# TritonDataCenter/dragnet

Measured on AMD Instinct MI355X. Metric: NDJSON records/sec (whole node), krill filter + 2-field breakdown (req.method,res.statusCode), higher is better.
Workload: dtype uint8; 1 GPU; model=dn scan: filter eq(req.method,GET) + breakdown req.method,res.statusCode, global_batch=4743501, seq_len=226, parallelism=dp1

## Files before the change

dragnet_amd/engine/gpu.py:

```python

import os
import stat
from types import SimpleNamespace

import numpy as np

from . import capacity, decode, xpose
from . import plan as planmod
from .chunks import _pad, choose_chunk_bytes, frame_files
from .decode import (
    C_DS_FAILEDEVAL, C_DS_FILTERED, C_GLOBAL_N, C_INVALID_JSON, C_LINES,
    C_OVERFLOW, C_PARSED, CM_AGG_IN, CM_BADDATE, CM_FAILEDEVAL,
    CM_FILTER_IN, CM_FILTERED, CM_N, CM_NONNUMERIC, CM_TIME_OUT, CM_UNDEF)
from .xpose import _build_xpose_layout


def _env_int(name, default):
    try:
        return int(os.environ.get(name, default))
    except ValueError:
        return default


def first_guess_slots():
    return (_env_int("DRAGNET_AGG_SLOTS", 1 << 20),
            _env_int("DRAGNET_DICT_SLOTS", 1 << 20))


def _is_regular(path):
    try:
        return stat.S_ISREG(os.stat(path).st_mode)
    except OSError:
        return False


class GpuEngine(object):
    name = "gpu"

    def __init__(self, device=None):
        import torch
        self.torch = torch
        if not torch.cuda.is_available():
            raise RuntimeError("no GPU visible (torch.cuda unavailable)")
        from ..ops import load_ops
        self.ops = load_ops(required=True)
        self.device = device if device is not None else \
            torch.device("cuda", torch.cuda.current_device())
        self.chunk_bytes = _env_int("DRAGNET_CHUNK_MB", 256) * 1024 * 1024
        self.coded_stats = {"launches": 0, "retries": 0}
        if self.chunk_bytes > (3 << 30):
            raise ValueError(
                "DRAGNET_CHUNK_MB too large: device chunk addressing "
                "is 32-bit (max 3072 MB per chunk)")


    def scan(self, files, queries, ds_filter=None, time_field=None,
             data_format="json", byte_source=None):
        from ..datasource.file import ScanResult

        cplan = planmod.compile_plan(
            queries, ds_filter=ds_filter, time_field=time_field,
            data_format=data_format)

        agg_slots, dict_slots = first_guess_slots()
        dict_data = _env_int("DRAGNET_DICT_DATA_MB", 256) * 1024 * 1024

        if (byte_source is not None or _env_int("DRAGNET_GROW", 0) == 1
                or not all(_is_regular(p) for p in files)):
            ctx = _ScanContext(self, cplan, agg_slots, dict_slots,
                               dict_data, dense=False, growable=True)
            if byte_source is not None:
                for chunk in byte_source:
                    ctx.feed(chunk)
                ctx.flush()
            else:
                ctx.scan_files(files)
            if ctx.overflowed():
                raise RuntimeError(
                    "table overflow on non-restartable byte source")
            aggs, stages = ctx.finalize(queries)
            return ScanResult(aggs, stages, gpu_stats=dict(
                ctx.planner.grow_counts(), restarts=0))

        dense = None
        nogrow = {"agg": [0] * len(queries), "sdict": 0, "sdata": 0,
                  "ndict": 0}
        for attempt in range(4):
            ctx = _ScanContext(self, cplan, agg_slots, dict_slots,
                               dict_data, dense=dense)
            ctx.scan_files(files)
            if ctx.overflowed():
                from ..log import get_logger
                if ctx.dense:
                    get_logger().child("gpu-engine").warn(
                        "dense directory overflow; restarting on the "
                        "hash path", agg_slots=agg_slots)
                    dense = False
                    continue
                get_logger().child("gpu-engine").warn(
                    "aggregation table overflow; restarting scan",
                    agg_slots=agg_slots * 8, dict_slots=dict_slots * 8)
                dense = False
                agg_slots *= 8
                dict_slots *= 8
                dict_data *= 4
                continue
            aggs, stages = ctx.finalize(queries)
            return ScanResult(aggs, stages,
                              gpu_stats=dict(nogrow, restarts=attempt))
        raise RuntimeError("aggregation tables overflowed after retries")

    def columnar_query(self, query, filt, params, kinds, cols, vals):
        from . import colquery
        return colquery.columnar_query(self, query, filt, params, kinds,
                                       cols, vals)

    def coded_query(self, query, filt, params, kinds, merged,
                    timings=None):
        from . import colquery
        return colquery.coded_query(self, query, filt, params, kinds,
                                    merged, timings)


class _ScanContext(object):
    def __init__(self, eng, cplan, agg_slots, dict_slots, dict_data_cap,
                 dense=None, growable=False):
        torch = eng.torch
        if growable:
            dense = False
        self.eng = eng
        self.t = torch
        self.cplan = cplan
        dev = eng.device
        if dense is None:
            dense = _env_int("DRAGNET_DENSE", 1) == 1
        self.dense = dense
        if dense:
            agg_slots = _env_int("DRAGNET_DENSE_SLOTS", 8192)

        def dev_i32(np_arr):
            return torch.from_numpy(
                np.ascontiguousarray(np_arr.astype(np.int32))).to(dev)

        def dev_f64(np_arr):
            return torch.from_numpy(
                np.ascontiguousarray(np_arr.astype(np.float64))).to(dev)

        progs, bounds = cplan.programs
        metrics, sreq = cplan.metrics
        bds, steps = cplan.breakdown_descs
        plan = dict(
            field_sigs=torch.from_numpy(
                cplan.field_sigs.view(np.int64)).to(dev),
            comp_slot=torch.from_numpy(cplan.comp_slot).to(dev),
            nf_match=cplan.nf_match,
            sig_bloom=cplan.sig_bloom,
            fields_parent_sig=cplan.fields_parent_sig,
            prog_nodes=dev_i32(progs),
            prog_bounds=dev_i32(bounds),
            const_meta=dev_i32(cplan.const_meta),
            const_dvals=dev_f64(cplan.const_dvals),
            const_bytes=torch.from_numpy(
                np.ascontiguousarray(cplan.const_bytes)).to(dev),
            synth_slots=dev_i32(cplan.synthetic),
            n_synth=cplan.n_synth,
            metric_rows=dev_i32(metrics),
            synth_req=dev_i32(sreq),
            bd_rows=dev_i32(bds),
            bd_steps=dev_f64(steps),
            value_slot=cplan.value_slot,
            fields_slot=cplan.fields_slot,
            skinner=cplan.data_format == "json-skinner",
        )

        self.state = eng.ops.ScanState(
            plan=plan, agg_slots=agg_slots, dict_slots=dict_slots,
            dict_data_bytes=dict_data_cap, dense=dense)

        self.planner = None
        if growable:
            nm, s_cols, n_cols = capacity.plan_shape(metrics, bds)
            sizes = self.state.sizes()
            self.planner = capacity.CapacityPlanner(
                nm, s_cols, n_cols,
                dict(sizes, agg=[sizes["agg%d" % m] for m in range(nm)]))

        self._pinned = self._dev_data = None
        self._pos = self._nlines = self._segs = None
        self._partial = b""
        self._copy_ev = None
        self._fin_stream = None
        self._files = None
        self._pool = None
        self._x = None

    @property
    def counters(self):
        return self.state.counters

    @property
    def agg_slots(self):
        return max(v for k, v in self.state.sizes().items()
                   if k.startswith("agg"))

    @property
    def dict_slots(self):
        sizes = self.state.sizes()
        return max(sizes["sdict"], sizes["ndict"])


    def feed(self, chunk):
        data = self._partial + chunk
        cut = data.rfind(b"\n")
        if cut < 0:
            self._partial = data
            return
        self._partial = data[cut + 1:]
        self._run(data[:cut + 1])

    def flush(self):
        if self._partial:
            self._run(self._partial + b"\n")
            self._partial = b""

    def _ensure_buffers(self, padded):
        torch = self.t
        dev = self.eng.device
        if self._pinned is not None and self._pinned.numel() >= padded:
            return
        cap = max(padded, self.eng.chunk_bytes + (1 << 20))
        cap = (cap + 15) & ~15
        self._pinned = torch.empty(cap, dtype=torch.uint8, pin_memory=True)
        self._dev_data = torch.empty(cap, dtype=torch.uint8, device=dev)
        self._pos = torch.empty(cap + 2, dtype=torch.int32, device=dev)
        self._nlines = torch.zeros(1, dtype=torch.int32, device=dev)
        self._segs = torch.empty(cap // 2048 + 2, dtype=torch.int32,
                                 device=dev)

    @staticmethod
    def _pad_pinned(pin, n):
        padded = _pad(n)
        pin[n:padded] = 10
        return padded

    def _index(self, dev_data, start, end):
        self.eng.ops.newline_index(dev_data, start, end, self._segs,
                                   self._pos, self._nlines)
        return self._pos, self._nlines

    def _submit(self, dev_data, start, end, index=None):
        pos, nlines = index or self._index(dev_data, start, end)
        if self.planner is None:
            self.state.scan(dev_data, pos, nlines, start)
        else:
            self._scan_planned(dev_data, pos, nlines, start, end)


    def _scan_planned(self, dev_data, pos, nlines, start, end):
        torch = self.t
        pl = self.planner
        g = pl.floor
        host = torch.cat(
            [nlines, pos[g - 1:end - start:g]]).cpu().numpy()
        nrec = min(int(host[0]), pos.numel())
        marks = host[1:].view(np.uint32)

        def start_of(i):
            if i == 0:
                return start
            if i == nrec:
                return end
            return int(marks[i // g - 1]) + 1

        a = 0
        while a < nrec:
            b = pl.next_range(a, nrec, start_of, self._measure, self.grow)
            self.state.scan(dev_data, pos[a:b], nlines, start_of(a))
            a = b

    def _measure(self, names):
        occ = self.state.occupancy().cpu().tolist()
        true = dict(zip(self.planner.names, occ))
        return {n: true[n] for n in names}

    def grow(self, name, new_size):
        old = self.planner.size[name]
        if name.startswith("agg"):
            self.state.grow_agg(int(name[3:]), new_size)
        else:
            getattr(self.state, "grow_" + name)(new_size)
        self.planner.size[name] = new_size
        from ..log import get_logger
        get_logger().child("gpu-engine").warn(
            "table grown in place", structure=name, size=old,
            new_size=new_size)

    def _run(self, buf):
        torch = self.t
        n = len(buf)
        self._ensure_buffers(_pad(n))
        pin = self._pinned
        if self._copy_ev is None:
            self._copy_ev = torch.cuda.Event()
        else:
            self._copy_ev.synchronize()
        pin[:n] = torch.frombuffer(bytearray(buf), dtype=torch.uint8)
        padded = self._pad_pinned(pin, n)
        self._dev_data[:padded].copy_(pin[:padded], non_blocking=True)
        self._copy_ev.record()
        self._submit(self._dev_data, 0, n)

    def overflowed(self):
        return int(self.counters[C_OVERFLOW].item()) > 0


    def scan_files(self, files):
        cap = self.eng.chunk_bytes
        if self._pinned is None:
            try:
                total = sum(os.stat(p).st_size for p in files)
            except OSError:
                total = 0
            cap = choose_chunk_bytes(total, cap,
                                     "DRAGNET_CHUNK_MB" in os.environ)
        pins = self._ensure_file_staging(cap)
        evs = [None, None]

        def wait(i):
            if evs[i] is not None:
                evs[i].synchronize()
                evs[i] = None

        frames = frame_files(files, [memoryview(p.numpy()) for p in pins],
                             cap, wait, _env_int("DRAGNET_READERS", 24))
        try:
            for i, n in frames:
                evs[i] = self._run_pinned(pins[i], n)
        finally:
            frames.close()

    def _ensure_file_staging(self, cap):
        torch = self.t
        if self._files is None:
            if self._pinned is None:
                self._ensure_buffers(_pad(cap))
            self._files = SimpleNamespace(
                pins=[self._pinned, torch.empty(
                    self._pinned.numel(), dtype=torch.uint8,
                    pin_memory=True)],
                copy_stream=torch.cuda.Stream(device=self.eng.device),
                dev=[self._dev_data, torch.empty_like(self._dev_data)],
                done=[torch.cuda.Event(), torch.cuda.Event()],
                idx=0)
        return self._files.pins

    def _run_pinned(self, pin, n):
        torch = self.t
        f = self._files
        padded = self._pad_pinned(pin, n)
        idx = f.idx
        f.idx ^= 1
        dev_data = f.dev[idx]
        main = torch.cuda.current_stream(self.eng.device)
        cs = f.copy_stream
        cs.wait_event(f.done[idx])
        ev = torch.cuda.Event()
        with torch.cuda.stream(cs):
            dev_data[:padded].copy_(pin[:padded], non_blocking=True)
            ev.record(cs)
        main.wait_event(ev)
        self._submit(dev_data, 0, n)
        f.done[idx].record(main)
        return ev


    def stage_resident(self, buf, n_slices=None):
        torch = self.t
        if n_slices is None:
            n_slices = _env_int("DRAGNET_SLICES", 6)
        n = len(buf)
        self._ensure_buffers(_pad(n))
        pin = self._pinned
        pin[:n] = torch.frombuffer(bytearray(buf), dtype=torch.uint8)
        padded = self._pad_pinned(pin, n)

        bounds = sorted({0, n} | {buf.rfind(b"\n", 0, n * k // n_slices) + 1
                                  for k in range(1, n_slices)})
        slices = list(zip(bounds, bounds[1:]))
        self._pool = p = SimpleNamespace(
            n=n, padded=padded, slices=slices,
            copy_stream=torch.cuda.Stream(device=self.eng.device),
            evs=[torch.cuda.Event() for _ in slices],
            dev_pp=torch.empty_like(self._dev_data),
            pass_done=[torch.cuda.Event(), torch.cuda.Event()],
            idx=0, pos=[])

        self._dev_data[:padded].copy_(pin[:padded])
        for (s, e) in slices:
            pos, nlines = self._index(self._dev_data, s, e)
            p.pos.append(
                (pos[:int(nlines.item())].clone(), nlines.clone()))

    def scan_resident(self, h2d=True):
        torch = self.t
        p = self._pool
        padded = p.padded
        dev_data = self._dev_data
        pin = self._pinned
        main = torch.cuda.current_stream(self.eng.device)
        if h2d:
            idx = p.idx
            p.idx ^= 1
            dev_data = self._dev_data if idx == 0 else p.dev_pp
            ev_done = p.pass_done[idx]
            p.copy_stream.wait_event(ev_done)
            with torch.cuda.stream(p.copy_stream):
                for k, (s, e) in enumerate(p.slices):
                    s16 = s & ~15
                    e16 = min((e + 15) & ~15, padded)
                    dev_data[s16:e16].copy_(pin[s16:e16],
                                            non_blocking=True)
                    p.evs[k].record(p.copy_stream)
        for k, (s, e) in enumerate(p.slices):
            if h2d:
                main.wait_event(p.evs[k])
                self._submit(dev_data, s, e)
            else:
                self._submit(dev_data, s, e, p.pos[k])
        if h2d:
            ev_done.record(main)


    def stage_xpose(self, buf=None):
        gran = _env_int("DRAGNET_XGRAN", 64)
        if gran not in (32, 64, 128):
            raise ValueError("DRAGNET_XGRAN must be 32, 64 or 128")
        if os.environ.get("DRAGNET_XPOSE_HOST") == "1":
            self._x = xpose.build_on_host(self.t, buf, gran,
                                          self.eng.device)
            return
        if self._pool is None:
            if buf is None:
                raise ValueError("no resident pool to transpose")
            self.stage_resident(buf)
        pos, nlines = self._index(self._dev_data, 0, self._pool.n)
        self._x = xpose.build_on_device(self.t, self.eng.ops,
                                        self._dev_data, pos, nlines, gran)

    def scan_xpose(self):
        self.state.scan_xpose(*self._x)

    def make_graph(self, h2d=True, xpose=False):
        torch = self.t

        def pass_():
            self.reset()
            if xpose:
                self.scan_xpose()
            else:
                self.scan_resident(h2d=h2d)

        try:
            pass_()
            torch.cuda.synchronize(self.eng.device)
            g = torch.cuda.CUDAGraph()
            with torch.cuda.graph(g):
                pass_()
            torch.cuda.synchronize(self.eng.device)
            return g
        except Exception:
            return None

    def reset(self):
        self.state.reset()
        if self.planner is not None:
            self.planner.occ = dict.fromkeys(self.planner.names, 0)


    def finalize(self, queries):
        return self.decode_extracted(self.extract_async(queries),
                                     queries)

    def extract_async(self, queries):
        h = self.state.extract_all()
        h["ev"] = self.t.cuda.Event()
        h["ev"].record()
        return h

    def decode_extracted(self, h, queries):
        torch = self.t
        if self._fin_stream is None:
            self._fin_stream = torch.cuda.Stream(device=self.eng.device)
        with torch.cuda.stream(self._fin_stream):
            self._fin_stream.wait_event(h["ev"])
            host = {"cnt": h["cnt"].cpu().numpy()}
            host.update(self._fetch_dicts(h))
            host["aggs"] = []
            for k_full, c_full, out_n in h["aggs"][:len(queries)]:
                n_out = min(int(out_n.item()), k_full.shape[0])
                host["aggs"].append((k_full[:n_out].cpu().numpy(),
                                     c_full[:n_out].cpu().numpy()))
        return decode.decode_snapshot(host, queries, self.cplan)

    @staticmethod
    def _fetch_dicts(h):
        n_str = int(h["n_str"].item())
        n_num = int(h["n_num"].item())
        host = {"n_str": n_str, "n_num": n_num}
        if n_str:
            host["str_off"] = h["str_off"][:n_str].cpu().numpy()
            host["str_len"] = h["str_len"][:n_str].cpu().numpy()
            used = int(h["used"].item())
            host["blob"] = h["blob"][:used].cpu().numpy()
        if n_num:
            host["numbers"] = h["numbers"][:n_num].cpu().numpy()
        return host

    @classmethod
    def _decode_dicts(cls, h):
        return decode.decode_dicts(cls._fetch_dicts(h))
```

dragnet_amd/engine/plan.py:

```python


import os

import numpy as np

from .. import krill

FNV_OFFSET = 0xCBF29CE484222325
FNV_PRIME = 0x100000001B3
MASK64 = (1 << 64) - 1

OP_AND = 0
OP_OR = 1
OP_EQ = 2
OP_NE = 3
OP_LT = 4
OP_LE = 5
OP_GT = 6
OP_GE = 7
OP_TRUE = 8

CONST_NUM = 0
CONST_STR = 1
CONST_NULL = 2

BUCKET_NONE = 0
BUCKET_P2 = 1
BUCKET_LIN = 2

MAX_FIELDS = 24
MAX_DEPTH = 12
MAX_KEY = 8

(M_PROG, M_NBD, M_BD_OFF, M_NSYNTH, M_SYNTH_OFF, M_HAS_TF, M_T_GE,
 M_T_LT) = range(8)
M_N = 8


def fnv1a(data, h=FNV_OFFSET):
    for b in data:
        h = ((h ^ b) * FNV_PRIME) & MASK64
    return h


def _mix64(x):
    x &= MASK64
    x ^= x >> 33
    x = (x * 0xFF51AFD7ED558CCD) & MASK64
    x ^= x >> 33
    x = (x * 0xC4CEB9FE1A85EC53) & MASK64
    x ^= x >> 33
    return x


SIG_LENK = 0xFF51AFD7ED558CCD
SIG_LIT_MARK = 0xC2B2AE3D27D4EB4F


def _sig_mix(x):
    x &= MASK64
    x ^= x >> 32
    x = (x * 0xD6E8FEB86659FD93) & MASK64
    return x ^ (x >> 32)


def comp_into(sig, b):
    for k in range(0, len(b), 8):
        w = int.from_bytes(b[k:k + 8].ljust(8, b"\0"), "little")
        sig = _sig_mix(sig ^ w)
    return _sig_mix(sig ^ ((len(b) * SIG_LENK) & MASK64))


def lit_sig(name):
    return comp_into(FNV_OFFSET, name.encode("utf-8"))


def path_sig(path):
    sig = FNV_OFFSET
    for comp in path.split("."):
        sig = comp_into(sig, comp.encode("utf-8"))
    return sig


class PlanError(Exception):
    pass


class FieldTable(object):
    def __init__(self, prefix=""):
        self.prefix = prefix
        self.paths = []
        self.by_path = {}

    def slot(self, path, raw=False):
        key = (path, raw)
        if key in self.by_path:
            return self.by_path[key]
        i = len(self.paths)
        if i >= MAX_FIELDS:
            raise PlanError(
                "query references more than %d fields" % MAX_FIELDS)
        self.paths.append(key)
        self.by_path[key] = i
        return i

    def sigs(self):
        return np.array(
            [path_sig(p if raw else self.prefix + p)
             for p, raw in self.paths],
            dtype=np.uint64)


class ConstPool(object):
    def __init__(self):
        self.metas = []
        self.dvals = []
        self.bytes = bytearray()

    def add(self, v):
        if v is None:
            self.metas.append((CONST_NULL, 0, 0, 0))
            self.dvals.append(0.0)
        elif isinstance(v, bool):
            self.metas.append((CONST_NUM, 0, 0, 1))
            self.dvals.append(1.0 if v else 0.0)
        elif isinstance(v, (int, float)):
            self.metas.append((CONST_NUM, 0, 0, 1))
            self.dvals.append(float(v))
        else:
            import json as _json
            b = v.encode("utf-8")
            off = len(self.bytes)
            self.bytes.extend(b)
            num = krill.to_number(v)
            valid = 0 if num != num else 1
            esc = _json.dumps(v, ensure_ascii=False)[1:-1].encode("utf-8")
            if esc != b:
                off2 = len(self.bytes)
                self.bytes.extend(esc)
                alt = (off2, len(esc))
            else:
                alt = (0, 0)
            self.metas.append((CONST_STR, off, len(b), valid) + alt)
            self.dvals.append(num if valid else 0.0)
            return len(self.metas) - 1
        self.metas.append(self.metas.pop() + (0, 0))
        return len(self.metas) - 1


def compile_predicate(pred, fields, consts):
    nodes = []

    def emit(p):
        idx = len(nodes)
        if len(p) == 0:
            nodes.append([OP_TRUE, 0, 0, idx + 1])
            return
        (key, val), = p.items()
        if key == "and" or key == "or":
            nodes.append([OP_AND if key == "and" else OP_OR,
                          len(val), 0, 0])
            for sub in val:
                emit(sub)
            nodes[idx][3] = len(nodes)
            return
        op = {"eq": OP_EQ, "ne": OP_NE, "lt": OP_LT,
              "le": OP_LE, "gt": OP_GT, "ge": OP_GE}[key]
        slot = fields.slot(val[0])
        cidx = consts.add(val[1])
        nodes.append([op, slot, cidx, idx + 1])

    emit(pred if pred is not None else {})
    return nodes


class CompiledPlan(object):

    def __init__(self, fields, programs, const_meta, const_dvals,
                 const_bytes, synthetic, metrics, breakdown_descs,
                 queries):
        self.fields = fields
        self.field_sigs = fields.sigs()
        self.programs = programs
        self.const_meta = const_meta
        self.const_dvals = const_dvals
        self.const_bytes = const_bytes
        self.synthetic = synthetic
        self.metrics = metrics
        self.breakdown_descs = breakdown_descs
        self.queries = queries

    def describe(self):
        return {
            "fields": list(self.fields.paths),
            "n_metrics": int(self.metrics[0].shape[0]),
        }


def compile_plan(queries, ds_filter=None, time_field=None,
                 data_format="json"):
    prefix = "fields." if data_format == "json-skinner" else ""
    fields = FieldTable(prefix)
    consts = ConstPool()
    prog_nodes = []
    prog_bounds = []

    def add_program(pred):
        start = len(prog_nodes)
        nodes = compile_predicate(pred, fields, consts)
        for n in nodes:
            n[3] += start
        prog_nodes.extend(nodes)
        prog_bounds.append((start, len(prog_nodes)))
        return len(prog_bounds) - 1

    ds_prog = add_program(ds_filter)

    synth_slots = []
    synth_by_slot = {}

    def synth_index(src_path):
        slot = fields.slot(src_path)
        if slot in synth_by_slot:
            return synth_by_slot[slot]
        synth_by_slot[slot] = len(synth_slots)
        synth_slots.append(slot)
        return synth_by_slot[slot]

    metric_rows = []
    bd_rows = []
    bd_steps = []
    synth_req = []

    for q in queries:
        if len(q.breakdowns) > MAX_KEY:
            raise PlanError(
                "query has more than %d breakdowns (GPU key width); "
                "use the CPU engine" % MAX_KEY)
        prog_id = add_program(q.filter)

        my_synth = []
        for b in q.breakdowns:
            if "date" in b:
                my_synth.append(synth_index(b["field"]))
        has_tf = 0
        t_ge = t_lt = 0
        dn_ts_idx = -1
        if q.before_ms is not None:
            if not time_field:
                raise PlanError(
                    'datasource is missing "timefield" for "before" '
                    'and "after" constraints')
            dn_ts_idx = synth_index(time_field)
            my_synth.append(dn_ts_idx)
            has_tf = 1
            t_ge = -(-q.after_ms // 1000)
            t_lt = -(-q.before_ms // 1000)

        sreq_off = len(synth_req)
        seen = set()
        my_synth_u = [s for s in my_synth
                      if not (s in seen or seen.add(s))]
        synth_req.extend(my_synth_u)

        synth_names = {b["name"]: b["field"]
                       for b in q.breakdowns if "date" in b}
        if q.time_field:
            synth_names.setdefault(q.time_field, q.time_field)

        bd_off = len(bd_rows)
        for b in q.breakdowns:
            if "date" in b:
                kind = 1
                ref = synth_index(b["field"])
            elif b["name"] in synth_names:
                kind = 1
                ref = synth_index(synth_names[b["name"]])
            else:
                kind = 0
                ref = fields.slot(b["name"])
            bk = q.bucketizers.get(b["name"])
            if bk is None:
                bkind, step = BUCKET_NONE, 0.0
            elif bk.aggr == "quantize":
                bkind, step = BUCKET_P2, 0.0
            else:
                bkind, step = BUCKET_LIN, float(bk.step)
            bd_rows.append([kind, ref, bkind, 0])
            bd_steps.append(step)

        row = {M_PROG: prog_id, M_NBD: len(q.breakdowns),
               M_BD_OFF: bd_off, M_NSYNTH: len(my_synth_u),
               M_SYNTH_OFF: sreq_off, M_HAS_TF: has_tf,
               M_T_GE: int(t_ge), M_T_LT: int(t_lt)}
        metric_rows.append([row[c] for c in range(M_N)])

    value_slot = -1
    fields_slot = -1
    if data_format == "json-skinner":
        value_slot = fields.slot("value", raw=True)
        fields_slot = fields.slot("fields", raw=True)

    nf_match = len(fields.paths)
    comp_slot = np.full(max(nf_match, 1), -1, dtype=np.int32)
    comp_sigs = []
    no_companions = os.environ.get("DRAGNET_NO_COMPANIONS") == "1"
    if data_format != "json-skinner" and not no_companions:
        for i, (pth, raw) in enumerate(fields.paths):
            if not raw and "." in pth:
                phys = nf_match + len(comp_sigs)
                if phys >= MAX_FIELDS:
                    raise PlanError(
                        "query references more than %d fields "
                        "(incl. dotted-key companions)" % MAX_FIELDS)
                comp_slot[i] = phys
                comp_sigs.append(lit_sig(pth))
    elif data_format == "json-skinner" and not no_companions:
        for i, (pth, raw) in enumerate(fields.paths):
            if not raw and "." in pth:
                phys = nf_match + len(comp_sigs)
                if phys >= MAX_FIELDS:
                    raise PlanError(
                        "query references more than %d fields "
                        "(incl. dotted-key companions)" % MAX_FIELDS)
                comp_slot[i] = phys
                comp_sigs.append(_sig_mix(
                    path_sig(prefix + pth) ^ SIG_LIT_MARK))

    programs = np.array(prog_nodes, dtype=np.int32).reshape(-1, 4)
    bounds = np.array(prog_bounds, dtype=np.int32).reshape(-1, 2)
    const_meta = np.array(consts.metas, dtype=np.int32).reshape(-1, 6)
    const_dvals = np.array(consts.dvals, dtype=np.float64)
    const_bytes = np.frombuffer(
        bytes(consts.bytes) or b"\0", dtype=np.uint8).copy()
    synthetic = np.array(synth_slots or [0], dtype=np.int32)
    metrics = np.array(metric_rows, dtype=np.int32).reshape(-1, M_N)
    bds = np.array(bd_rows or [[0, 0, 0, 0]],
                   dtype=np.int32).reshape(-1, 4)
    steps = np.array(bd_steps or [0.0], dtype=np.float64)
    sreq = np.array(synth_req or [0], dtype=np.int32)

    plan = CompiledPlan(
        fields, (programs, bounds), const_meta, const_dvals,
        const_bytes, synthetic, (metrics, sreq), (bds, steps), queries)
    plan.n_synth = len(synth_slots)
    plan.comp_slot = comp_slot
    plan.nf_match = nf_match
    bloom = 0
    for sg in ([int(x) for x in fields.sigs()] + comp_sigs):
        bloom |= 1 << (sg & 63)
    plan.sig_bloom = bloom - (1 << 64) if bloom >= (1 << 63) else bloom
    if comp_sigs:
        plan.field_sigs = np.concatenate(
            [plan.field_sigs,
             np.array(comp_sigs, dtype=np.uint64)])
    plan.value_slot = value_slot
    plan.fields_slot = fields_slot
    fps = path_sig("fields") if data_format == "json-skinner" else 0
    plan.fields_parent_sig = fps - (1 << 64) if fps >= (1 << 63) else fps
    plan.ds_prog = ds_prog
    plan.data_format = data_format
    return plan



TAG_ORD = 0
TAG_STR = 1
TAG_NUM = 2
TAG_SPECIAL = 3
ORD_BIAS = 1 << 29
SPECIAL_NULL = 0
SPECIAL_UNDEF = 1
SPECIAL_TRUE = 2
SPECIAL_FALSE = 3
SPECIAL_OBJECT = 4
SPECIAL_ARRAY = 5
SPECIAL_ARRJSON = 6
EMPTY_CODE = 0xFFFFFFFF


def decode_key(codes, query, strings, numbers):
    from ..points import js_num_str
    out = []
    for b, code in zip(query.breakdowns, codes):
        tag = code >> 30
        val = code & 0x3FFFFFFF
        bk = query.bucketizers.get(b["name"])
        if bk is not None:
            if tag == TAG_ORD:
                out.append(int(val) - ORD_BIAS)
            else:
                assert tag == TAG_NUM
                out.append(int(numbers[val]))
        elif tag == TAG_STR:
            out.append(strings[val])
        elif tag == TAG_NUM:
            num = numbers[val]
            if "date" in b:
                out.append(int(num))
            else:
                out.append(js_num_str(
                    int(num) if float(num).is_integer()
                    and abs(num) < 2**53 else float(num)))
        elif tag == TAG_SPECIAL:
            if (val & 7) == SPECIAL_ARRJSON:
                import json as _json
                from ..points import js_array_str
                raw = strings[val >> 3]
                try:
                    out.append(js_array_str(_json.loads(raw)))
                except ValueError:
                    out.append(raw)
            else:
                out.append({
                    SPECIAL_NULL: "null", SPECIAL_UNDEF: "undefined",
                    SPECIAL_TRUE: "true", SPECIAL_FALSE: "false",
                    SPECIAL_OBJECT: "[object Object]",
                    SPECIAL_ARRAY: "<array>"}[val])
        else:
            raise PlanError("bad code tag %d" % tag)
    return tuple(out)
```

dragnet_amd/ops/hip/common.h:

```cpp
#pragma once
#if defined(__HIPCC__)
#include <hip/hip_runtime.h>
#endif
#include <cstddef>
#include <cstdint>
#include "hd.h"

namespace dn {

constexpr int MAX_FIELDS = 24;
constexpr int MAX_DEPTH  = 64;
constexpr int SLOT_DEPTH = 12;
constexpr int MAX_KEY    = 8;
constexpr int MAX_SYNTH  = 8;
constexpr int PRED_STACK = 8;

enum PredOp : int32_t {
  OP_AND = 0, OP_OR = 1,
  OP_EQ = 2, OP_NE = 3, OP_LT = 4, OP_LE = 5, OP_GT = 6, OP_GE = 7,
  OP_TRUE = 8,
};

enum ConstKind : int32_t { CONST_NUM = 0, CONST_STR = 1, CONST_NULL = 2 };

enum BucketKind : int32_t { BUCKET_NONE = 0, BUCKET_P2 = 1, BUCKET_LIN = 2 };

enum FieldType : uint8_t {
  T_MISSING = 0, T_NULL = 1, T_FALSE = 2, T_TRUE = 3,
  T_NUM = 4, T_STR = 5, T_OBJ = 6, T_ARR = 7,
};

constexpr uint32_t TAG_ORD     = 0u;
constexpr uint32_t TAG_STR     = 1u;
constexpr uint32_t TAG_NUM     = 2u;
constexpr uint32_t TAG_SPECIAL = 3u;
constexpr uint32_t ORD_BIAS    = 1u << 29;
constexpr uint32_t SPECIAL_NULL = 0, SPECIAL_UNDEF = 1,
                   SPECIAL_TRUE = 2, SPECIAL_FALSE = 3,
                   SPECIAL_OBJECT = 4, SPECIAL_ARRAY = 5,
                   SPECIAL_ARRJSON = 6;
constexpr uint32_t EMPTY_CODE = 0xFFFFFFFFu;

inline DN_HD uint32_t make_code(uint32_t tag, uint32_t val) {
  return (tag << 30) | (val & 0x3FFFFFFFu);
}

enum CounterSlot : int {
  C_LINES = 0,
  C_INVALID_JSON = 1,
  C_PARSED = 2,
  C_DS_FILTERED = 3,
  C_DS_FAILEDEVAL = 4,
  C_OVERFLOW = 5,
  C_GLOBAL_N = 8,
  CM_FILTER_IN = 0, CM_FILTERED = 1, CM_FAILEDEVAL = 2,
  CM_UNDEF = 3, CM_BADDATE = 4, CM_TIME_OUT = 5,
  CM_AGG_IN = 6, CM_NONNUMERIC = 7,
  CM_N = 8,
};

constexpr uint32_t SLOT_EMPTY = 0, SLOT_CLAIMED = 1, SLOT_READY = 2;

struct AggTable {
  uint32_t* state;
  uint32_t* keys;
  double*   count;
  uint32_t  nslots;
  double*   partial;
  uint32_t  prows;
  uint32_t  pad_;
};

struct StrDict {
  uint32_t* state;
  uint64_t* hash;
  uint32_t* id;
  uint32_t* off;
  uint32_t* len;
  uint32_t  nslots;
  uint8_t*  data;
  uint32_t  data_cap;
  uint32_t* data_used;
  uint32_t* next_id;
};

struct NumDict {
  uint32_t* state;
  uint64_t* bits;
  uint32_t* id;
  uint32_t  nslots;
  uint32_t* next_id;
};


struct PlanView {
  const uint64_t* field_sigs;
  int nf;
  const int32_t* comp_slot;
  int nf_match;
  uint64_t sig_bloom;
  const int32_t* prog_nodes;
  const int32_t* prog_bounds;
  const int32_t* const_meta;
  const double*  const_dvals;
  const uint8_t* const_bytes;
  const int32_t* synth_slots;
  int ns;
  const int32_t* metric_rows;
  const int32_t* synth_req;
  const int32_t* bd_rows;
  const double*  bd_steps;
  int nm;
  int value_slot;
  int fields_slot;
  uint64_t fields_parent_sig;
};

struct ScanArgs {
  const uint8_t* data;
  const uint32_t* nl_pos;
  const uint32_t* nlines_ptr;
  uint32_t pos_cap;
  uint32_t first_start;
  uint32_t tile_cap;
  PlanView P;
  AggTable* tables;
  StrDict sdict;
  NumDict ndict;
  unsigned long long* counters;
  int data_format_skinner;
  const uint8_t* xdata;
  const unsigned long long* xwave_base;
  const uint32_t* xrec_len;
  uint32_t xn_slots;
};

}
```

dragnet_amd/ops/hip/ext.hip:

```cpp

#include <torch/extension.h>
#include <cstdlib>
#include <cstring>
#include <c10/hip/HIPStream.h>

#include "scan_kernels.hip"

namespace dn {

namespace {

#define CHECK_GPU(t) TORCH_CHECK((t).is_cuda(), #t " must be on GPU")

constexpr size_t LDS_MAX = 160 * 1024;

hipStream_t current_stream() {
  return c10::hip::getCurrentHIPStream().stream();
}

template <class... KArgs, class... Args>
void launch(const char* what, void (*kernel)(KArgs...), dim3 grid,
            dim3 block, size_t lds, Args&&... args) {
  hipLaunchKernelGGL(kernel, grid, block, lds, current_stream(),
                     std::forward<Args>(args)...);
  hipError_t err = hipGetLastError();
  TORCH_CHECK(err == hipSuccess, what, " launch failed: ",
              hipGetErrorString(err));
}

constexpr uint32_t GRID_CAP = 2048;

uint32_t grid_for(uint64_t n) {
  return (uint32_t)std::min<uint64_t>((n + BLOCK - 1) / BLOCK, GRID_CAP);
}

int env_int(const char* name, int dflt) {
  const char* v = getenv(name);
  return v ? atoi(v) : dflt;
}

size_t lds_bytes(int64_t nf, int64_t nm, int64_t ns, bool columnar) {
  return LdsLayout((int)nf, (int)nm, columnar ? 0 : (int)ns, !columnar)
      .total;
}

using ScanKernel = void (*)(ScanArgs);

ScanKernel linear_kernel(int mw) {
  switch (mw) {
    case 2: return scan_kernel_mw<2>;
    case 3: return scan_kernel_mw<3>;
    case 4: return scan_kernel_mw<4>;
    case 5: return scan_kernel_mw<5>;
    case 6: return scan_kernel_mw<6>;
    default: return scan_kernel;
  }
}

ScanKernel xpose_kernel(int mw, int xg) {
  if (xg == 32) return scan_kernel_x<4, 5>;
  if (xg == 128) return scan_kernel_x<4, 7>;
  switch (mw) {
    case 2: return scan_kernel_x<2, 6>;
    case 3: return scan_kernel_x<3, 6>;
    case 5: return scan_kernel_x<5, 6>;
    default: return scan_kernel_x<4, 6>;
  }
}

}

void newline_index(torch::Tensor data, int64_t start, int64_t n,
                   torch::Tensor seg_scratch,
                   torch::Tensor pos_out, torch::Tensor total_out) {
  CHECK_GPU(data);
  int64_t span = n - (start & ~(int64_t)15);
  uint32_t nseg = (uint32_t)((span + NL_SEG - 1) / NL_SEG);
  TORCH_CHECK((int64_t)nseg <= seg_scratch.numel(),
              "seg_scratch too small");
  if (span <= 0) {
    total_out.zero_();
    return;
  }
  const uint8_t* d = (const uint8_t*)data.data_ptr();
  uint32_t* segs = (uint32_t*)seg_scratch.data_ptr();
  uint32_t blocks = (nseg + 3) / 4;
  launch("newline_count", newline_count_kernel, dim3(blocks), dim3(256), 0,
         d, (uint32_t)start, (uint32_t)n, segs, nseg);
  launch("newline_scan", newline_scan_kernel, dim3(1), dim3(1024), 0,
         segs, nseg, (uint32_t*)total_out.data_ptr());
  launch("newline_write", newline_write_kernel, dim3(blocks), dim3(256), 0,
         d, (uint32_t)start, (uint32_t)n, segs, nseg,
         (uint32_t*)pos_out.data_ptr(), (uint32_t)pos_out.numel());
}

torch::Tensor col_descs_host(std::vector<int64_t> kinds,
                             std::vector<torch::Tensor> nums,
                             std::vector<torch::Tensor> soffs,
                             std::vector<torch::Tensor> slens) {
  int nf = (int)kinds.size();
  auto out = torch::zeros({(long)(nf * sizeof(ColDesc))},
                          torch::dtype(torch::kUInt8));
  ColDesc* d = (ColDesc*)out.data_ptr();
  for (int f = 0; f < nf; f++) {
    d[f].kind = (int32_t)kinds[f];
    d[f].num = kinds[f] == COL_NUM ? (const double*)nums[f].data_ptr()
                                   : nullptr;
    d[f].soff = (kinds[f] == COL_STR || kinds[f] == COL_CODED)
                    ? (const uint32_t*)soffs[f].data_ptr()
                    : nullptr;
    d[f].slen = kinds[f] == COL_STR ? (const uint32_t*)slens[f].data_ptr()
                                    : nullptr;
  }
  return out;
}

void xpose_build(torch::Tensor data, torch::Tensor sstart,
                 torch::Tensor slen, torch::Tensor wbase,
                 int64_t n_slots, int64_t gran_log, torch::Tensor xb) {
  CHECK_GPU(data);
  CHECK_GPU(xb);
  uint32_t nw = (uint32_t)(n_slots >> 6);
  TORCH_CHECK(wbase.numel() >= (long)nw + 1, "wbase needs nw+1 rows");
  uint32_t blocks = (nw + 3) / 4;
  launch("xpose_build", xpose_build_kernel, dim3(blocks), dim3(256), 0,
         (const uint8_t*)data.data_ptr(),
         (const uint32_t*)sstart.data_ptr(),
         (const uint32_t*)slen.data_ptr(),
         (const unsigned long long*)wbase.data_ptr(),
         (uint32_t)n_slots, (int)gran_log, (uint8_t*)xb.data_ptr());
}

class ScanState {
 public:
  ScanState(py::dict plan, int64_t agg_slots, int64_t dict_slots,
            int64_t dict_data_bytes, bool dense)
      : dense_(dense) {
    auto ptr = [&](py::dict& d, const char* key) {
      owned_.push_back(py::cast<torch::Tensor>(d[key]));
      return owned_.back().data_ptr();
    };
    PlanView& P = args_.P;
    P.field_sigs = (const uint64_t*)ptr(plan, "field_sigs");
    P.nf = (int)owned_.back().numel();
    P.comp_slot = (const int32_t*)ptr(plan, "comp_slot");
    P.nf_match = py::cast<int>(plan["nf_match"]);
    P.sig_bloom = (uint64_t)py::cast<int64_t>(plan["sig_bloom"]);
    P.prog_nodes = (const int32_t*)ptr(plan, "prog_nodes");
    P.prog_bounds = (const int32_t*)ptr(plan, "prog_bounds");
    P.const_meta = (const int32_t*)ptr(plan, "const_meta");
    P.const_dvals = (const double*)ptr(plan, "const_dvals");
    P.const_bytes = (const uint8_t*)ptr(plan, "const_bytes");
    P.synth_slots = (const int32_t*)ptr(plan, "synth_slots");
    P.ns = py::cast<int>(plan["n_synth"]);
    P.metric_rows = (const int32_t*)ptr(plan, "metric_rows");
    P.nm = (int)(owned_.back().numel() / 8);
    P.synth_req = (const int32_t*)ptr(plan, "synth_req");
    P.bd_rows = (const int32_t*)ptr(plan, "bd_rows");
    P.bd_steps = (const double*)ptr(plan, "bd_steps");
    P.value_slot = py::cast<int>(plan["value_slot"]);
    P.fields_slot = py::cast<int>(plan["fields_slot"]);
    P.fields_parent_sig =
        (uint64_t)py::cast<int64_t>(plan["fields_parent_sig"]);
    args_.data_format_skinner = py::cast<bool>(plan["skinner"]) ? 1 : 0;

    for (auto& t : owned_) CHECK_GPU(t);
    device_ = owned_.front().device();

    check_slots(agg_slots, "agg table", AGG_LOG2);
    check_slots(dict_slots, "sdict", DICT_LOG2);
    check_bytes(dict_data_bytes);
    states_.resize(P.nm);
    keys_.resize(P.nm);
    counts_.resize(P.nm);
    if (dense_) partials_.resize(P.nm);
    for (int m = 0; m < P.nm; m++) alloc_agg(m, agg_slots);
    alloc_sdict(dict_slots);
    alloc_ndict(dict_slots);
    sd_data_ = zeros({dict_data_bytes}, U8);
    sd_used_ = zeros({1}, I32);
    sd_next_ = zeros({1}, I32);
    nd_next_ = zeros({1}, I32);
    counters_ = zeros({C_GLOBAL_N + P.nm * CM_N}, I64);
    bind_tables();
    bind_dicts();
    args_.counters = (unsigned long long*)counters_.data_ptr();

    int mw = env_int("DRAGNET_MIN_WAVES", 4);
    linear_ = linear_kernel(mw);
    xpose_ = xpose_kernel(mw, env_int("DRAGNET_XGRAN", 64));

    lds_ = lds_bytes(P.nf, P.nm, P.ns, false);
    TORCH_CHECK(lds_ <= LDS_MAX, "plan needs too much LDS: ", lds_);
    int tile_req = env_int("DRAGNET_LDS_STAGE", 0);
    if (tile_req != 0) {
      size_t avail = (LDS_MAX - lds_ - 256) & ~(size_t)15;
      tile_cap_ = (tile_req < 0) ? avail
                                 : std::min((size_t)tile_req, avail);
      if (tile_cap_ > 100 * 1024) tile_cap_ = 100 * 1024;
      if (tile_cap_ < 24 * 1024) tile_cap_ = 0;
    }
    args_.tile_cap = (uint32_t)tile_cap_;
  }

  void scan(torch::Tensor data, torch::Tensor nl_pos,
            torch::Tensor nlines, int64_t first_start) {
    CHECK_GPU(data);
    CHECK_GPU(nl_pos);
    ScanArgs A = args_;
    A.data = (const uint8_t*)data.data_ptr();
    A.nl_pos = (const uint32_t*)nl_pos.data_ptr();
    A.nlines_ptr = (const uint32_t*)nlines.data_ptr();
    A.pos_cap = (uint32_t)nl_pos.numel();
    A.first_start = (uint32_t)first_start;
    launch("scan_kernel", linear_, dim3(grid_for(A.pos_cap)), dim3(BLOCK),
           lds_ + tile_cap_, A);
  }

  void scan_xpose(torch::Tensor xdata, torch::Tensor wave_base,
                  torch::Tensor rec_len, int64_t n_slots) {
    CHECK_GPU(xdata);
    TORCH_CHECK(n_slots > 0, "empty transposed staging");
    ScanArgs A = args_;
    A.xdata = (const uint8_t*)xdata.data_ptr();
    A.xwave_base = (const unsigned long long*)wave_base.data_ptr();
    A.xrec_len = (const uint32_t*)rec_len.data_ptr();
    A.xn_slots = (uint32_t)n_slots;
    launch("scan_kernel_x", xpose_, dim3(grid_for(A.xn_slots)),
           dim3(BLOCK), lds_ + tile_cap_, A);
  }

  void columnar_query(torch::Tensor col_descs, torch::Tensor blob,
                      torch::Tensor values, int64_t nrows,
                      std::vector<torch::Tensor> columns) {
    ColumnLaunch L = bind_columns("columnar", col_descs, blob, values,
                                  nrows, std::move(columns));
    if (L.blocks == 0) return;
    launch("columnar_query", columnar_query_kernel, dim3(L.blocks),
           dim3(BLOCK), L.lds, L.A);
  }

  void coded_query(torch::Tensor col_descs, torch::Tensor dict_blob,
                   torch::Tensor doff, torch::Tensor dlen,
                   torch::Tensor seg_start, torch::Tensor values,
                   int64_t nrows, std::vector<torch::Tensor> columns) {
    for (auto* t : {&doff, &dlen, &seg_start}) CHECK_GPU(*t);
    TORCH_CHECK(doff.numel() == dlen.numel(), "doff / dlen differ");
    TORCH_CHECK(doff.numel() < (int64_t)0xFFFFFFFFll, "dictionary too big");
    TORCH_CHECK(seg_start.numel() >= 2 &&
                    seg_start.numel() - 1 < (int64_t)ORD_BIAS,
                "seg_start needs nfiles + 1 entries");
    ColumnLaunch L = bind_columns("coded", col_descs, dict_blob, values,
                                  nrows, std::move(columns));
    auto code2id = zeros({std::max<int64_t>(doff.numel(), 1)}, I32);
    col_inputs_.insert(col_inputs_.end(),
                       {doff, dlen, seg_start, code2id});
    CodedArgs X;
    X.ndict = (uint32_t)doff.numel();
    X.nfiles = (uint32_t)(seg_start.numel() - 1);
    X.doff = (const uint32_t*)doff.data_ptr();
    X.dlen = (const uint32_t*)dlen.data_ptr();
    X.code2id = (const uint32_t*)code2id.data_ptr();
    X.seg_start = (const uint32_t*)seg_start.data_ptr();
    if (X.ndict > 0)
      launch("dict_intern", dict_intern_kernel,
             dim3((X.ndict + 255) / 256), dim3(256), 0, L.A.sdict, L.A.blob,
             X.doff, X.dlen, X.ndict, (uint32_t*)code2id.data_ptr(),
             overflow_ptr());
    if (L.blocks == 0) return;
    launch("coded_query", coded_query_kernel, dim3(L.blocks), dim3(BLOCK),
           L.lds, L.A, X);
  }

  void reset() {
    hipStream_t st = current_stream();
    auto z = [&](torch::Tensor& t) {
      hipError_t e = hipMemsetAsync(t.data_ptr(), 0,
                                    (size_t)t.numel() * t.element_size(),
                                    st);
      TORCH_CHECK(e == hipSuccess, "reset memset failed: ",
                  hipGetErrorString(e));
    };
    for (auto& t : states_) z(t);
    for (auto& t : counts_) z(t);
    for (auto& t : partials_) z(t);
    z(sd_state_); z(sd_used_); z(sd_next_);
    z(nd_state_); z(nd_next_); z(counters_);
  }

  py::dict extract_all() {
    for (const AggTable& T : tables_) dense_reduce(T);
    const StrDict& sd = args_.sdict;
    const NumDict& nd = args_.ndict;
    py::dict out;
    out["cnt"] = counters_.clone();
    out["n_str"] = sd_next_.clone();
    out["n_num"] = nd_next_.clone();
    out["used"] = sd_used_.clone();
    out["blob"] = sd_data_.clone();

    long n_sids = std::max<long>(sd.nslots, 1);
    auto str_off = zeros({n_sids}, I32);
    auto str_len = zeros({n_sids}, I32);
    if (sd.nslots > 0)
      launch("extract_strdict", extract_strdict_kernel,
             dim3((sd.nslots + 255) / 256), dim3(256), 0, sd,
             (uint32_t*)str_off.data_ptr(), (uint32_t*)str_len.data_ptr(),
             sd.nslots);
    out["str_off"] = str_off;
    out["str_len"] = str_len;

    auto numbers = zeros({std::max<long>(nd.nslots, 1)}, F64);
    if (nd.nslots > 0)
      launch("extract_numdict", extract_numdict_kernel,
             dim3((nd.nslots + 255) / 256), dim3(256), 0, nd,
             (double*)numbers.data_ptr(), nd.nslots);
    out["numbers"] = numbers;

    py::list aggs;
    for (const AggTable& T : tables_) {
      long max_out = T.nslots;
      auto out_keys = zeros({max_out, (long)MAX_KEY}, I32);
      auto out_counts = zeros({max_out}, F64);
      auto out_n = zeros({1}, I32);
      launch("extract_agg", extract_agg_kernel,
             dim3((T.nslots + 255) / 256), dim3(256), 0, T,
             (uint32_t*)out_keys.data_ptr(),
             (double*)out_counts.data_ptr(), (uint32_t*)out_n.data_ptr(),
             (uint32_t)max_out);
      aggs.append(py::make_tuple(out_keys, out_counts, out_n));
    }
    out["aggs"] = aggs;
    return out;
  }

  py::dict sizes() const {
    py::dict out;
    for (size_t m = 0; m < tables_.size(); m++)
      out[py::str("agg" + std::to_string(m))] = tables_[m].nslots;
    out["sdict"] = args_.sdict.nslots;
    out["sdata"] = args_.sdict.data_cap;
    out["ndict"] = args_.ndict.nslots;
    return out;
  }

  torch::Tensor counters() const { return counters_; }


  torch::Tensor occupancy() {
    std::vector<torch::Tensor> parts;
    for (auto& st : states_)
      parts.push_back(st.eq((int64_t)SLOT_READY).sum().reshape({1}));
    for (auto* t : {&sd_next_, &sd_used_, &nd_next_})
      parts.push_back(t->to(torch::kInt64));
    return torch::cat(parts);
  }

  void grow_agg(int64_t m, int64_t new_slots) {
    TORCH_CHECK(!dense_, "dense tables do not grow");
    TORCH_CHECK(m >= 0 && (size_t)m < tables_.size(), "no such metric");
    AggTable old = tables_[m];
    check_slots(new_slots, "agg table", AGG_LOG2, old.nslots);
    std::vector<torch::Tensor> keep = {states_[m], keys_[m], counts_[m]};
    growing("agg" + std::to_string(m), old.nslots, new_slots,
            [&] { alloc_agg(m, new_slots); });
    bind_tables();
    launch("rehash_agg", rehash_agg_kernel, dim3((old.nslots + 255) / 256),
           dim3(256), 0, old, tables_[m], overflow_ptr());
  }

  void grow_sdict(int64_t new_slots) {
    StrDict old = args_.sdict;
    check_slots(new_slots, "sdict", DICT_LOG2, old.nslots);
    std::vector<torch::Tensor> keep = {sd_state_, sd_hash_, sd_id_,
                                       sd_off_, sd_len_};
    growing("sdict", old.nslots, new_slots, [&] { alloc_sdict(new_slots); });
    bind_dicts();
    launch("rehash_strdict", rehash_strdict_kernel,
           dim3((old.nslots + 255) / 256), dim3(256), 0, old, args_.sdict,
           overflow_ptr());
  }

  void grow_sdata(int64_t new_bytes) {
    torch::Tensor old = sd_data_;
    check_bytes(new_bytes, old.numel());
    growing("sdata", old.numel(), new_bytes,
            [&] { sd_data_ = zeros({new_bytes}, U8); });
    bind_dicts();
    hipError_t e = hipMemcpyAsync(
        sd_data_.data_ptr(), old.data_ptr(), (size_t)old.numel(),
        hipMemcpyDeviceToDevice, current_stream());
    TORCH_CHECK(e == hipSuccess, "payload copy failed: ",
                hipGetErrorString(e));
  }

  void grow_ndict(int64_t new_slots) {
    NumDict old = args_.ndict;
    check_slots(new_slots, "ndict", DICT_LOG2, old.nslots);
    std::vector<torch::Tensor> keep = {nd_state_, nd_bits_, nd_id_};
    growing("ndict", old.nslots, new_slots, [&] { alloc_ndict(new_slots); });
    bind_dicts();
    launch("rehash_numdict", rehash_numdict_kernel,
           dim3((old.nslots + 255) / 256), dim3(256), 0, old, args_.ndict,
           overflow_ptr());
  }

 private:
  static constexpr auto I32 = torch::kInt32, I64 = torch::kInt64,
                        F64 = torch::kFloat64, U8 = torch::kUInt8;

  torch::Tensor zeros(at::IntArrayRef shape, torch::ScalarType dtype) const {
    return torch::zeros(shape, torch::dtype(dtype).device(device_));
  }

  static constexpr int DICT_LOG2 = 31, AGG_LOG2 = 29;
  static void check_slots(int64_t n, const char* what, int max_log2,
                          int64_t old = 0) {
    TORCH_CHECK(n > 0 && (n & (n - 1)) == 0 && (n >> max_log2) <= 1, what,
                ": slot count must be a power of two <= 2^", max_log2);
    TORCH_CHECK(n > old, "a table may only grow (", old, " -> ", n,
                " slots)");
  }

  static void check_bytes(int64_t n, int64_t old = -1) {
    TORCH_CHECK(n <= (int64_t)0xFFFFFFFFll,
                "string payload buffer exceeds 32-bit offsets");
    TORCH_CHECK(n > old, "string payload buffer may only grow");
  }

  template <class Alloc>
  static void growing(const std::string& name, int64_t old_size,
                      int64_t new_size, Alloc&& alloc) {
    try {
      alloc();
    } catch (const c10::OutOfMemoryError& e) {
      std::string why = e.what_without_backtrace();
      TORCH_CHECK(false, "cannot grow ", name, " from ", old_size, " to ",
                  new_size, ": device allocation failed (",
                  why.substr(0, why.find('\n')), ")");
    }
  }

  struct ColumnLaunch {
    ColArgs A;
    size_t lds;
    uint32_t blocks;
  };

  ColumnLaunch bind_columns(const char* what, torch::Tensor col_descs,
                            torch::Tensor blob, torch::Tensor values,
                            int64_t nrows,
                            std::vector<torch::Tensor> columns) {
    for (auto* t : {&col_descs, &blob, &values}) CHECK_GPU(*t);
    for (auto& t : columns) {
      CHECK_GPU(t);
      TORCH_CHECK(t.numel() >= nrows, "column shorter than nrows");
    }
    TORCH_CHECK(nrows >= 0 && nrows < (int64_t)0xFFFFFFFFll, what,
                " query: row count exceeds 32 bits");
    TORCH_CHECK(values.numel() >= nrows, "values shorter than nrows");
    ColumnLaunch L;
    ColArgs& A = L.A;
    A.P = column_plan();
    TORCH_CHECK(col_descs.numel() == (int64_t)(A.P.nf * sizeof(ColDesc)),
                "col_descs does not match the plan's field count");
    L.lds = lds_bytes(A.P.nf, A.P.nm, 0, true);
    TORCH_CHECK(L.lds <= LDS_MAX, what, " plan needs too much LDS");
    A.nrows = (uint32_t)nrows;
    A.values = (const double*)values.data_ptr();
    A.blob = (const uint8_t*)blob.data_ptr();
    A.cols = (const ColDesc*)col_descs.data_ptr();
    A.tables = args_.tables;
    A.sdict = args_.sdict;
    A.ndict = args_.ndict;
    A.counters = args_.counters;
    col_inputs_ = std::move(columns);
    col_inputs_.insert(col_inputs_.end(), {col_descs, blob, values});
    L.blocks = grid_for((uint64_t)nrows);
    return L;
  }

  PlanView column_plan() const {
    PlanView P = args_.P;
    P.sig_bloom = 0;
    P.fields_parent_sig = 0;
    P.ns = 0;
    P.value_slot = -1;
    P.fields_slot = -1;
    return P;
  }

  unsigned long long* overflow_ptr() {
    return (unsigned long long*)counters_.data_ptr() + C_OVERFLOW;
  }

  void alloc_agg(size_t m, int64_t n) {
    std::tie(states_[m], keys_[m], counts_[m]) = std::make_tuple(
        zeros({n}, I32), zeros({n * MAX_KEY}, I32), zeros({n}, F64));
    if (dense_) partials_[m] = zeros({GRID_CAP, n}, F64);
  }

  void alloc_sdict(int64_t n) {
    std::tie(sd_state_, sd_hash_, sd_id_, sd_off_, sd_len_) =
        std::make_tuple(zeros({n}, I32), zeros({n}, I64), zeros({n}, I32),
                        zeros({n}, I32), zeros({n}, I32));
  }

  void alloc_ndict(int64_t n) {
    std::tie(nd_state_, nd_bits_, nd_id_) =
        std::make_tuple(zeros({n}, I32), zeros({n}, I64), zeros({n}, I32));
  }

  void bind_dicts() {
    StrDict& sd = args_.sdict;
    sd.state = (uint32_t*)sd_state_.data_ptr();
    sd.hash = (uint64_t*)sd_hash_.data_ptr();
    sd.id = (uint32_t*)sd_id_.data_ptr();
    sd.off = (uint32_t*)sd_off_.data_ptr();
    sd.len = (uint32_t*)sd_len_.data_ptr();
    sd.nslots = (uint32_t)sd_state_.numel();
    sd.data = (uint8_t*)sd_data_.data_ptr();
    sd.data_cap = (uint32_t)sd_data_.numel();
    sd.data_used = (uint32_t*)sd_used_.data_ptr();
    sd.next_id = (uint32_t*)sd_next_.data_ptr();
    NumDict& nd = args_.ndict;
    nd.state = (uint32_t*)nd_state_.data_ptr();
    nd.bits = (uint64_t*)nd_bits_.data_ptr();
    nd.id = (uint32_t*)nd_id_.data_ptr();
    nd.nslots = (uint32_t)nd_state_.numel();
    nd.next_id = (uint32_t*)nd_next_.data_ptr();
  }

  void bind_tables() {
    size_t nm = states_.size();
    tables_.resize(nm);
    for (size_t m = 0; m < nm; m++) {
      AggTable& t = tables_[m];
      t.state = (uint32_t*)states_[m].data_ptr();
      t.keys = (uint32_t*)keys_[m].data_ptr();
      t.count = (double*)counts_[m].data_ptr();
      t.nslots = (uint32_t)states_[m].numel();
      t.partial = dense_ ? (double*)partials_[m].data_ptr() : nullptr;
      t.prows = dense_ ? GRID_CAP : 0;
      t.pad_ = 0;
    }
    auto host = torch::empty({(long)(nm * sizeof(AggTable))},
                             torch::dtype(torch::kUInt8));
    memcpy(host.data_ptr(), tables_.data(), nm * sizeof(AggTable));
    table_descs_ = host.to(device_);
    args_.tables = (AggTable*)table_descs_.data_ptr();
  }

  static void dense_reduce(const AggTable& T) {
    if (T.partial == nullptr || T.prows == 0) return;
    uint32_t tiles = (T.nslots + 15) / 16;
    uint32_t splits = 32;
    while (splits > 1 && T.prows / splits < 16) splits /= 2;
    uint32_t rows_per_blk = (T.prows + splits - 1) / splits;
    rows_per_blk = (rows_per_blk + 3) & ~3u;
    launch("mfma_reduce", mfma_reduce_kernel, dim3(tiles, splits),
           dim3(64), 0, T, rows_per_blk);
  }

  std::vector<torch::Tensor> states_, keys_, counts_, partials_, owned_;
  std::vector<torch::Tensor> col_inputs_;
  torch::Tensor sd_state_, sd_hash_, sd_id_, sd_off_, sd_len_;
  torch::Tensor sd_data_, sd_used_, sd_next_;
  torch::Tensor nd_state_, nd_bits_, nd_id_, nd_next_;
  torch::Tensor counters_, table_descs_;
  c10::Device device_ = c10::kCPU;
  const bool dense_;
  ScanArgs args_ = {};
  std::vector<AggTable> tables_;
  ScanKernel linear_ = nullptr, xpose_ = nullptr;
  size_t lds_ = 0, tile_cap_ = 0;
};

}

PYBIND11_MODULE(TORCH_EXTENSION_NAME, m) {
  m.doc() = "dragnet_amd MI355X scan engine (gfx950 HIP kernels)";
  m.def("newline_index", &dn::newline_index, "device-side newline index");
  m.def("xpose_build", &dn::xpose_build, "device-side wave transpose");
  m.def("col_descs_host", &dn::col_descs_host);
  m.def("lds_bytes", &dn::lds_bytes, py::arg("nf"), py::arg("nm"),
        py::arg("ns") = 0, py::arg("columnar") = false,
        "dynamic LDS bytes of a scan / columnar launch (host only)");
  py::class_<dn::ScanState>(m, "ScanState")
      .def(py::init<py::dict, int64_t, int64_t, int64_t, bool>(),
           py::kw_only(), py::arg("plan"), py::arg("agg_slots"),
           py::arg("dict_slots"), py::arg("dict_data_bytes"),
           py::arg("dense"))
      .def("scan", &dn::ScanState::scan, py::arg("data"),
           py::arg("nl_pos"), py::arg("nlines"), py::arg("first_start"),
           "fused NDJSON scan over one chunk")
      .def("scan_xpose", &dn::ScanState::scan_xpose, py::arg("xdata"),
           py::arg("wave_base"), py::arg("rec_len"), py::arg("n_slots"))
      .def("columnar_query", &dn::ScanState::columnar_query,
           py::arg("col_descs"), py::arg("blob"), py::arg("values"),
           py::arg("nrows"), py::arg("columns"),
           "K7: query over uploaded index columns")
      .def("coded_query", &dn::ScanState::coded_query,
           py::arg("col_descs"), py::arg("dict_blob"), py::arg("doff"),
           py::arg("dlen"), py::arg("seg_start"), py::arg("values"),
           py::arg("nrows"), py::arg("keep"),
           "query over merged dictionary-coded sidecar columns")
      .def("reset", &dn::ScanState::reset)
      .def("extract_all", &dn::ScanState::extract_all)
      .def("occupancy", &dn::ScanState::occupancy,
           "device int64 [ready slots per metric..., string ids, "
           "payload bytes, number ids]")
      .def("sizes", &dn::ScanState::sizes)
      .def_property_readonly("counters", &dn::ScanState::counters)
      .def("grow_agg", &dn::ScanState::grow_agg, py::arg("metric"),
           py::arg("new_slots"),
           "rehash one metric's table into a larger zeroed one")
      .def("grow_sdict", &dn::ScanState::grow_sdict, py::arg("new_slots"))
      .def("grow_sdata", &dn::ScanState::grow_sdata, py::arg("new_bytes"))
      .def("grow_ndict", &dn::ScanState::grow_ndict, py::arg("new_slots"));
  m.attr("MAX_KEY") = (int)dn::MAX_KEY;
  m.attr("MAX_FIELDS") = (int)dn::MAX_FIELDS;
}
```

dragnet_amd/ops/hip/hd.h:

```cpp
#pragma once

#if defined(__HIPCC__)
#define DN_HD __host__ __device__
#define DN_HD_INLINE __host__ __device__ __forceinline__
#define DN_HD_NOINLINE __host__ __device__ __attribute__((noinline))
#else
#define DN_HD
#define DN_HD_INLINE inline
#define DN_HD_NOINLINE __attribute__((noinline))
#endif

#if defined(__HIP_DEVICE_COMPILE__)
#define DN_FFSLL(x) __ffsll(x)
#define DN_DOUBLE_AS_LL(x) __double_as_longlong(x)
#define DN_LL_AS_DOUBLE(x) __longlong_as_double(x)
#define DN_TID() ((uint32_t)threadIdx.x)
#define DN_CONST_TABLE __device__ __constant__
#else
#define DN_FFSLL(x) __builtin_ffsll((long long)(x))
#define DN_DOUBLE_AS_LL(x) __builtin_bit_cast(long long, (double)(x))
#define DN_LL_AS_DOUBLE(x) __builtin_bit_cast(double, (long long)(x))
#define DN_TID() 0u
#define DN_CONST_TABLE static const
#endif
```

dragnet_amd/ops/hip/scan_kernels.hip:

```cpp

#include "common.h"
#include <hip/hip_runtime.h>

extern "C++" {
#include "scan_text.h"
#include "scan_record.h"
#include "scan_tables.h"

namespace dn {

typedef double dn_d4 __attribute__((ext_vector_type(4)));

__global__ void mfma_reduce_kernel(AggTable T, uint32_t rows_per_blk) {
  uint32_t slot0 = blockIdx.x * 16;
  uint32_t r0 = blockIdx.y * rows_per_blk;
  uint32_t r1 = r0 + rows_per_blk;
  if (r1 > T.prows) r1 = T.prows;
  int l = threadIdx.x;
  uint32_t n = slot0 + (l & 15);
  dn_d4 acc = {0.0, 0.0, 0.0, 0.0};
  const double* P = T.partial;
  size_t stride = T.nslots;
  for (uint32_t rt = r0; rt < r1; rt += 4) {
    uint32_t rr = rt + (uint32_t)(l >> 4);
    double b = (rr < r1 && n < T.nslots)
                   ? P[(size_t)rr * stride + n] : 0.0;
    acc = __builtin_amdgcn_mfma_f64_16x16x4f64(1.0, b, acc, 0, 0, 0);
  }
  if (l < 16 && n < T.nslots) {
    double v = acc[0];
    if (v != 0.0) atomicAdd(&T.count[n], v);
  }
}


constexpr uint32_t NL_SEG = 2048;

DEV uint32_t nl_mask32(uint32_t w) {
  uint32_t x = w ^ 0x0A0A0A0Au;
  uint32_t y = (x & 0x7F7F7F7Fu) + 0x7F7F7F7Fu;
  return ~(y | x | 0x7F7F7F7Fu);
}

DEV uint32_t range_mask32(uint32_t wpos, uint32_t start, uint32_t n) {
  uint32_t m = 0x80808080u;
  if (wpos >= start && wpos + 4 <= n) return m;
  uint32_t out = 0;
#pragma unroll
  for (int b = 0; b < 4; b++) {
    uint32_t pos = wpos + b;
    if (pos >= start && pos < n) out |= 0x80u << (b * 8);
  }
  return out;
}

__global__ void newline_count_kernel(const uint8_t* data,
                                     uint32_t start, uint32_t n,
                                     uint32_t* seg_counts,
                                     uint32_t nseg) {
  uint32_t seg = blockIdx.x * (blockDim.x >> 6) + (threadIdx.x >> 6);
  if (seg >= nseg) return;
  uint32_t lane = threadIdx.x & 63u;
  const uint4* p16 = reinterpret_cast<const uint4*>(data);
  uint32_t base0 = (start & ~15u) + seg * NL_SEG;
  uint32_t cnt = 0;
#pragma unroll
  for (int half = 0; half < 2; half++) {
    uint32_t base = base0 + half * 1024u + lane * 16u;
    if (base < n) {
      uint4 v = p16[base >> 4];
      uint32_t w[4] = {v.x, v.y, v.z, v.w};
#pragma unroll
      for (int wi = 0; wi < 4; wi++)
        cnt += __popc(nl_mask32(w[wi]) &
                      range_mask32(base + wi * 4, start, n));
    }
  }
  for (int off = 32; off; off >>= 1) cnt += __shfl_down(cnt, off, 64);
  if (lane == 0) seg_counts[seg] = cnt;
}

__global__ void newline_scan_kernel(uint32_t* seg_counts, uint32_t nseg,
                                    uint32_t* total_out) {
  __shared__ uint32_t tile[1024];
  __shared__ uint32_t carry;
  if (threadIdx.x == 0) carry = 0;
  __syncthreads();
  for (uint32_t base = 0; base < nseg; base += 1024) {
    uint32_t i = base + threadIdx.x;
    uint32_t v = (i < nseg) ? seg_counts[i] : 0;
    tile[threadIdx.x] = v;
    __syncthreads();
    for (uint32_t d = 1; d < 1024; d <<= 1) {
      uint32_t t = (threadIdx.x >= d) ? tile[threadIdx.x - d] : 0;
      __syncthreads();
      tile[threadIdx.x] += t;
      __syncthreads();
    }
    uint32_t incl = tile[threadIdx.x];
    if (i < nseg) seg_counts[i] = carry + incl - v;
    __syncthreads();
    if (threadIdx.x == 1023) carry += tile[1023];
    __syncthreads();
  }
  if (threadIdx.x == 0) *total_out = carry;
}

__global__ void newline_write_kernel(const uint8_t* data,
                                     uint32_t start, uint32_t n,
                                     const uint32_t* seg_offsets,
                                     uint32_t nseg, uint32_t* out_pos,
                                     uint32_t cap) {
  uint32_t seg = blockIdx.x * (blockDim.x >> 6) + (threadIdx.x >> 6);
  if (seg >= nseg) return;
  uint32_t lane = threadIdx.x & 63u;
  const uint4* p16 = reinterpret_cast<const uint4*>(data);
  uint32_t base0 = (start & ~15u) + seg * NL_SEG;
  uint32_t w_at = seg_offsets[seg];
#pragma unroll
  for (int half = 0; half < 2; half++) {
    uint32_t base = base0 + half * 1024u + lane * 16u;
    uint32_t m[4] = {0, 0, 0, 0};
    uint32_t cnt = 0;
    if (base < n) {
      uint4 v = p16[base >> 4];
      uint32_t w[4] = {v.x, v.y, v.z, v.w};
#pragma unroll
      for (int wi = 0; wi < 4; wi++) {
        m[wi] = nl_mask32(w[wi]) &
                range_mask32(base + wi * 4, start, n);
        cnt += __popc(m[wi]);
      }
    }
    uint32_t incl = cnt;
    for (int off = 1; off < 64; off <<= 1) {
      uint32_t t = __shfl_up(incl, off, 64);
      if ((int)lane >= off) incl += t;
    }
    uint32_t at = w_at + incl - cnt;
#pragma unroll
    for (int wi = 0; wi < 4; wi++) {
      uint32_t mm = m[wi];
      while (mm) {
        uint32_t b = ((uint32_t)__ffs(mm) - 1) >> 3;
        if (at < cap) out_pos[at] = base + wi * 4 + b;
        at++;
        mm &= mm - 1;
      }
    }
    w_at += __shfl(incl, 63, 64);
  }
}

__global__ void xpose_build_kernel(const uint8_t* __restrict__ data,
                                   const uint32_t* __restrict__ sstart,
                                   const uint32_t* __restrict__ slen,
                                   const unsigned long long* __restrict__ wbase,
                                   uint32_t n_slots, int gran_log,
                                   uint8_t* __restrict__ xb) {
  uint32_t w = blockIdx.x * (blockDim.x >> 6) + (threadIdx.x >> 6);
  uint32_t nw = n_slots >> 6;
  if (w >= nw) return;
  uint32_t lane = threadIdx.x & 63u;
  uint32_t r = (w << 6) + lane;
  uint32_t gran = 1u << gran_log;
  unsigned long long base = wbase[w];
  uint32_t gw = (uint32_t)((wbase[w + 1] - base) >> (6 + gran_log));
  uint32_t len = slen[r];
  if (len == 0xFFFFFFFFu) len = 0;
  uint32_t start = sstart[r];
  uint8_t* dst0 = xb + base + ((size_t)lane << gran_log);
  for (uint32_t g = 0; g < gw; g++) {
    uint8_t* dst = dst0 + ((size_t)g << (6 + gran_log));
    uint32_t off = g << gran_log;
    for (uint32_t k = 0; k < gran; k += 16) {
      uint8_t tmp[16];
#pragma unroll
      for (int t = 0; t < 16; t++) {
        uint32_t o = off + k + t;
        tmp[t] = (o < len) ? data[start + o] : (uint8_t)'\n';
      }
      uint4 vv;
      __builtin_memcpy(&vv, tmp, 16);
      *reinterpret_cast<uint4*>(dst + k) = vv;
    }
  }
}

template <int XP>
DEV void scan_kernel_body(char* smem, ScanArgs A);

__launch_bounds__(BLOCK)
__global__ void scan_kernel(ScanArgs A) {
  extern __shared__ __attribute__((aligned(16))) char smem0[];
  scan_kernel_body<0>(smem0, A);
}

template <int MW>
__launch_bounds__(BLOCK, MW)
__global__ void scan_kernel_mw(ScanArgs A) {
  extern __shared__ __attribute__((aligned(16))) char smem1[];
  scan_kernel_body<0>(smem1, A);
}
template __global__ void scan_kernel_mw<2>(ScanArgs);
template __global__ void scan_kernel_mw<3>(ScanArgs);
template __global__ void scan_kernel_mw<4>(ScanArgs);
template __global__ void scan_kernel_mw<5>(ScanArgs);
template __global__ void scan_kernel_mw<6>(ScanArgs);

template <int MW, int XLG>
__launch_bounds__(BLOCK, MW)
__global__ void scan_kernel_x(ScanArgs A) {
  extern __shared__ __attribute__((aligned(16))) char smem2[];
  scan_kernel_body<XLG>(smem2, A);
}
template __global__ void scan_kernel_x<2, 6>(ScanArgs);
template __global__ void scan_kernel_x<3, 6>(ScanArgs);
template __global__ void scan_kernel_x<4, 6>(ScanArgs);
template __global__ void scan_kernel_x<5, 6>(ScanArgs);
template __global__ void scan_kernel_x<4, 5>(ScanArgs);
template __global__ void scan_kernel_x<4, 7>(ScanArgs);

#define synth_val_at(si) synth_lds[(si) * BLOCK + threadIdx.x]

template <class BS>
DEV void process_record(BS BV, uint32_t start, uint32_t end,
                        const ScanArgs& A, const PlanView& P, FV& fv,
                        unsigned long long* lcnt, LdsCacheEntry* cache,
                        uint64_t* sig_lds, double* synth_lds) {
  const int nf = P.nf;
  uint32_t synth_ok = 0;
  atomicAdd(&lcnt[C_LINES], 1ull);
  for (int f = 0; f < nf; f++)
    fv.type[f * BLOCK + fv.tid] = T_MISSING;

  uint8_t top_type;
  bool ok = (end > start) &&
            parse_record(BV, start, end, P, fv, top_type, sig_lds,
                         A.data_format_skinner);
  double weight = 1.0;
  if (ok && A.data_format_skinner) {
    bool has_fields = P.fields_slot >= 0 &&
                      fv.get_type(P.fields_slot) != T_MISSING;
    bool val_num = P.value_slot >= 0 &&
                   fv.get_type(P.value_slot) == T_NUM;
    if (top_type != T_OBJ || !has_fields || !val_num) ok = false;
    else weight = fv.get_num(P.value_slot);
  }
  if (!ok) {
    atomicAdd(&lcnt[C_INVALID_JSON], 1ull);
  } else {
    atomicAdd(&lcnt[C_PARSED], 1ull);

    int keep = eval_predicate(P, BV, fv, 0);
    if (keep == -1) atomicAdd(&lcnt[C_DS_FAILEDEVAL], 1ull);
    else if (keep == 0) atomicAdd(&lcnt[C_DS_FILTERED], 1ull);

    if (keep == 1) {
      synth_ok = 0;
      for (int si = 0; si < P.ns; si++) {
        int slot = P.synth_slots[si];
        uint8_t t = fv.get_type(slot);
        uint32_t ok;
        if (t == T_MISSING) ok = 2;
        else if (t == T_NUM) {
          ok = 1; synth_val_at(si) = fv.get_num(slot);
        } else if (t == T_STR) {
          DateOut d = parse_iso_ms(BV, fv.get_soff(slot),
                                   fv.get_slen(slot));
          if (d.ok) {
            long long secs = d.ms >= 0 ? d.ms / 1000
                                       : (d.ms - 999) / 1000;
            ok = 1; synth_val_at(si) = (double)secs;
          } else ok = 3;
        } else ok = 3;
        synth_ok |= ok << (2 * si);
      }

      for (int m = 0; m < P.nm; m++) {
        const int32_t* M = &P.metric_rows[m * 8];
        unsigned long long* mc = &lcnt[C_GLOBAL_N + m * CM_N];
        atomicAdd(&mc[CM_FILTER_IN], 1ull);

        int res = eval_predicate(P, BV, fv, M[0]);
        if (res == -1) { atomicAdd(&mc[CM_FAILEDEVAL], 1ull); continue; }
        if (res == 0) { atomicAdd(&mc[CM_FILTERED], 1ull); continue; }

        bool sok = true;
        for (int k = 0; k < M[3]; k++) {
          int si = P.synth_req[M[4] + k];
          uint32_t ok = (synth_ok >> (2 * si)) & 3u;
          if (ok != 1) {
            atomicAdd(&mc[ok == 2 ? CM_UNDEF : CM_BADDATE], 1ull);
            sok = false; break;
          }
        }
        if (!sok) continue;

        if (M[5]) {
          int si = P.synth_req[M[4] + M[3] - 1];
          double ts = synth_val_at(si);
          if (!(ts >= (double)M[6] && ts < (double)M[7])) {
            atomicAdd(&mc[CM_TIME_OUT], 1ull); continue;
          }
        }

        atomicAdd(&mc[CM_AGG_IN], 1ull);

        uint32_t key[MAX_KEY];
        int nk = M[1];
        bool drop = false, overflow = false;
        for (int bi = 0; bi < nk; bi++) {
          const int32_t* B = &P.bd_rows[(M[2] + bi) * 4];
          double step = P.bd_steps[M[2] + bi];
          uint8_t t; double num = 0.0; uint32_t so = 0, sl = 0;
          if (B[0] == 1) {
            int si = B[1];
            if (((synth_ok >> (2 * si)) & 3u) == 1) {
              t = T_NUM; num = synth_val_at(si);
            } else t = T_MISSING;
          } else {
            int slot = B[1];
            int cs2 = P.comp_slot[slot];
            if (cs2 >= 0 && fv.get_type(cs2) != T_MISSING)
              slot = cs2;
            t = fv.get_type(slot);
            num = fv.get_num(slot);
            so = fv.get_soff(slot); sl = fv.get_slen(slot);
          }
          uint32_t code;
          if (!encode_key_col(A.sdict, A.ndict, BV, t, num, so, sl, B[2],
                              step, code, drop, overflow))
            break;
#pragma unroll
          for (int kk = 0; kk < MAX_KEY; kk++)
            if (kk == bi) key[kk] = code;
        }
        if (overflow) { atomicAdd(&lcnt[C_OVERFLOW], 1ull); continue; }
        if (drop) { atomicAdd(&mc[CM_NONNUMERIC], 1ull); continue; }
#pragma unroll
        for (int k = 0; k < MAX_KEY; k++)
          if (k >= nk) key[k] = 0;

        uint64_t kh = agg_key_hash(m, key);

        if (!A.data_format_skinner) {
          uint64_t unproc = __ballot(true);
          bool leader = false;
          double wsum = 0.0;
          while (unproc) {
            int src = (int)(__ffsll((long long)unproc) - 1);
            uint64_t src_kh = __shfl(kh, src);
            bool same = (kh == src_kh);
            uint64_t grp = __ballot(same);
            if (same && __lane_id() == src) {
              leader = true;
              wsum = (double)__popcll(grp);
            }
            unproc &= ~grp;
          }
          if (!leader) continue;
          weight = wsum;
        }
        lds_cache_add<1>(cache, A.tables, A.counters, lcnt, m, key, nk, kh,
                      weight);
      }
    }
  }
}

template <int XP>
DEV void scan_kernel_body(char* smem, ScanArgs A) {
  const PlanView& P = A.P;
  const int nf = P.nf;

  const LdsLayout L(nf, P.nm, P.ns, true);
  LdsCacheEntry* cache = reinterpret_cast<LdsCacheEntry*>(smem + L.cache);
  unsigned long long* lcnt =
      reinterpret_cast<unsigned long long*>(smem + L.lcnt);
  const int NCNT = C_GLOBAL_N + P.nm * CM_N;
  double* synth_lds = reinterpret_cast<double*>(smem + L.synth);
  uint64_t* sig_lds = reinterpret_cast<uint64_t*>(smem + L.sig);
  uint8_t* tile = reinterpret_cast<uint8_t*>(smem + L.tile);
  block_agg_init(cache, lcnt, NCNT);

  FV fv;
  fv.type = reinterpret_cast<uint8_t*>(smem + L.fv_type);
  fv.soff = reinterpret_cast<uint32_t*>(smem + L.fv_soff);
  fv.slen = reinterpret_cast<uint32_t*>(smem + L.fv_slen);
  fv.tid = threadIdx.x;

  if constexpr (XP != 0) {
    const uint32_t stride_x = gridDim.x * BLOCK;
    for (uint32_t rbase = blockIdx.x * BLOCK; rbase < A.xn_slots;
         rbase += stride_x) {
      uint32_t r = rbase + threadIdx.x;
      if (r < A.xn_slots) {
        uint32_t len = A.xrec_len[r];
        if (len != 0xFFFFFFFFu) {
          XBytesT<XP> BV;
          BV.base = A.xdata + A.xwave_base[r >> 6]
                    + ((size_t)(r & 63u) << XP);
          process_record(BV, 0u, len, A, P, fv, lcnt, cache, sig_lds,
                         synth_lds);
        }
      }
    }
  } else {
  uint32_t nlines = *A.nlines_ptr;
  if (nlines > A.pos_cap) nlines = A.pos_cap;
  const uint32_t stride = gridDim.x * BLOCK;
  for (uint32_t rbase = blockIdx.x * BLOCK; rbase < nlines;
       rbase += stride) {
    uint32_t r = rbase + threadIdx.x;
    bool active = r < nlines;

    Bytes BV;
    BV.mem = A.data;
    BV.bias = 0;
    uint32_t t_start = rbase ? A.nl_pos[rbase - 1] + 1 : A.first_start;
    uint32_t r_last = rbase + BLOCK - 1;
    if (r_last >= nlines) r_last = nlines - 1;
    uint32_t t_end = A.nl_pos[r_last] + 1;
    uint32_t t_base = t_start & ~15u;
    uint32_t span = t_end - t_base;
    bool staged = A.tile_cap >= 16 && span <= A.tile_cap;
    if (staged) {
      const uint4* g16 = reinterpret_cast<const uint4*>(A.data + t_base);
      uint4* l16 = reinterpret_cast<uint4*>(tile);
      uint32_t n16 = (span + 15) >> 4;
      for (uint32_t i = threadIdx.x; i < n16; i += BLOCK)
        l16[i] = g16[i];
      __syncthreads();
      BV.mem = tile;
      BV.bias = t_base;
    }

    if (active) {
      uint32_t start = r ? A.nl_pos[r - 1] + 1 : A.first_start;
      uint32_t end = A.nl_pos[r];
      process_record(BV, start, end, A, P, fv, lcnt, cache, sig_lds,
                     synth_lds);
    }

    if (staged) __syncthreads();
  }
  }

  block_agg_flush(cache, lcnt, NCNT, P, A.tables, A.counters);
}


__global__ void extract_agg_kernel(AggTable T, uint32_t* out_keys,
                                   double* out_counts, uint32_t* out_n,
                                   uint32_t max_out) {
  uint32_t s = blockIdx.x * blockDim.x + threadIdx.x;
  if (s >= T.nslots) return;
  if (atomic_load_relaxed(&T.state[s]) != SLOT_READY) return;
  uint32_t i = atomicAdd(out_n, 1u);
  if (i >= max_out) return;
  for (int k = 0; k < MAX_KEY; k++)
    out_keys[i * MAX_KEY + k] = T.keys[s * MAX_KEY + k];
  out_counts[i] = T.count[s];
}

__global__ void extract_strdict_kernel(StrDict D, uint32_t* out_off,
                                       uint32_t* out_len, uint32_t max_ids) {
  uint32_t s = blockIdx.x * blockDim.x + threadIdx.x;
  if (s >= D.nslots) return;
  if (atomic_load_relaxed(&D.state[s]) != SLOT_READY) return;
  uint32_t id = D.id[s];
  if (id >= max_ids) return;
  out_off[id] = D.off[s];
  out_len[id] = D.len[s];
}

__global__ void extract_numdict_kernel(NumDict D, double* out_vals,
                                       uint32_t max_ids) {
  uint32_t s = blockIdx.x * blockDim.x + threadIdx.x;
  if (s >= D.nslots) return;
  if (atomic_load_relaxed(&D.state[s]) != SLOT_READY) return;
  uint32_t id = D.id[s];
  if (id >= max_ids) return;
  out_vals[id] = __longlong_as_double(
      (long long)atomic_load_relaxed(&D.bits[s]));
}

}

#include "scan_rehash.h"

#include "scan_columns.h"

}
```

dragnet_amd/ops/hip/scan_record.h:

```cpp
#pragma once
#include "scan_text.h"

namespace dn {

constexpr int BLOCK = 256;
constexpr int SIG_DEPTH = 6;


struct FV {
  uint8_t* type;
  uint32_t* soff;
  uint32_t* slen;
  int tid;
  DN_HD_INLINE void set(int f, uint8_t t, uint32_t off, uint32_t len,
                        double n) {
    type[f * BLOCK + tid] = t;
    if (t == T_NUM) {
      uint64_t b = (uint64_t)DN_DOUBLE_AS_LL(n);
      soff[f * BLOCK + tid] = (uint32_t)b;
      slen[f * BLOCK + tid] = (uint32_t)(b >> 32);
    } else {
      soff[f * BLOCK + tid] = off;
      slen[f * BLOCK + tid] = len;
    }
  }
  DN_HD_INLINE void set_len(int f, uint32_t len) {
    slen[f * BLOCK + tid] = len;
  }
  DN_HD_INLINE uint8_t get_type(int f) const { return type[f * BLOCK + tid]; }
  DN_HD_INLINE uint32_t get_soff(int f) const { return soff[f * BLOCK + tid]; }
  DN_HD_INLINE uint32_t get_slen(int f) const { return slen[f * BLOCK + tid]; }
  DN_HD_INLINE double get_num(int f) const {
    uint64_t b = (uint64_t)soff[f * BLOCK + tid]
               | ((uint64_t)slen[f * BLOCK + tid] << 32);
    return DN_LL_AS_DOUBLE((long long)b);
  }
};


template <class BS>
DN_HD_INLINE bool parse_record(BS BV, uint32_t start, uint32_t end,
                               const PlanView& P, FV& fv, uint8_t& top_type,
                               uint64_t* sig_lds, bool dot_splits) {
  CursorT<BS> c; c.init(BV, start, end);
  #define sig_stack_at(d) sig_lds[(d) * BLOCK + DN_TID()]

  uint64_t cont_slot = ~0ull;
  uint64_t is_arr_bits = 0;
  int depth = 0;
  int arr_depth = 0;
  uint64_t cur_sig = 0;
  bool cur_capture = false;
  int cur_slot = -1;

  c.skip_ws();
  if (c.eof()) return false;

  auto match_slot = [&](uint64_t sig) -> int {
    if (!((P.sig_bloom >> ((uint32_t)sig & 63u)) & 1ull)) return -1;
    for (int f = 0; f < P.nf; f++)
      if (P.field_sigs[f] == sig) return f;
    return -1;
  };

  auto parse_key = [&](uint64_t parent, bool root, uint64_t& sig_out) -> bool {
    if (c.eof() || c.next() != '"') return false;
    int r = scan_key_sig(c, root ? FNV_OFFSET : parent, sig_out,
                         dot_splits);
    if (r == 0) return false;
    if (r == 2 && !root && parent == P.fields_parent_sig)
      sig_out = sig_mix(sig_out ^ SIG_LIT_MARK);
    return true;
  };

  bool expect_value = true;
  top_type = T_MISSING;

  while (true) {
    if (expect_value) {
      c.skip_ws();
      if (c.eof()) return false;
      uint8_t b = c.peek();
      uint8_t vtype = T_MISSING;
      uint32_t voff = 0, vlen = 0;
      double vnum = 0.0;

      if (b == '{') {
        uint32_t vstart = c.pos;
        c.pos++;
        if (cur_capture && arr_depth == 0)
          fv.set(cur_slot, T_OBJ, vstart, 0, 0.0);
        if (depth == 0) top_type = T_OBJ;
        if (depth >= MAX_DEPTH) return false;
        c.skip_ws();
        if (!c.eof() && c.peek() == '}') {
          c.pos++;
          vtype = T_OBJ;
          voff = vstart; vlen = c.pos - vstart;
        } else {
          if (depth < SLOT_DEPTH) {
            uint64_t cs = (cur_capture && arr_depth == 0)
                              ? (uint64_t)cur_slot : 31ull;
            cont_slot = (cont_slot & ~(31ull << (5 * depth)))
                        | (cs << (5 * depth));
          }
          if (depth < SIG_DEPTH) sig_stack_at(depth) = cur_sig;
          is_arr_bits &= ~(1ull << depth);
          depth++;
          uint64_t ksig;
          if (!parse_key(cur_sig, depth == 1, ksig)) return false;
          c.skip_ws();
          if (c.eof() || c.next() != ':') return false;
          cur_sig = ksig;
          cur_slot = (arr_depth == 0) ? match_slot(ksig) : -1;
          cur_capture = cur_slot >= 0;
          continue;
        }
      } else if (b == '[') {
        uint32_t vstart = c.pos;
        c.pos++;
        if (cur_capture && arr_depth == 0)
          fv.set(cur_slot, T_ARR, vstart, 0, 0.0);
        if (depth == 0) top_type = T_ARR;
        if (depth >= MAX_DEPTH) return false;
        c.skip_ws();
        if (!c.eof() && c.peek() == ']') {
          c.pos++;
          vtype = T_ARR;
          voff = vstart; vlen = c.pos - vstart;
        } else {
          if (depth < SLOT_DEPTH) {
            uint64_t cs = (cur_capture && arr_depth == 0)
                              ? (uint64_t)cur_slot : 31ull;
            cont_slot = (cont_slot & ~(31ull << (5 * depth)))
                        | (cs << (5 * depth));
          }
          if (depth < SIG_DEPTH) sig_stack_at(depth) = cur_sig;
          is_arr_bits |= (1ull << depth);
          depth++;
          arr_depth++;
          cur_capture = false; cur_slot = -1;
          continue;
        }
      } else if (b == '"') {
        c.pos++;
        if (!scan_string_fast(c, voff, vlen)) return false;
        vtype = T_STR;
      } else if (b == 't') {
        if (c.end - c.pos < 4) return false;
        if (c.byte_at(c.pos+1)!='r'||c.byte_at(c.pos+2)!='u'||c.byte_at(c.pos+3)!='e') return false;
        c.pos += 4; vtype = T_TRUE;
      } else if (b == 'f') {
        if (c.end - c.pos < 5) return false;
        if (c.byte_at(c.pos+1)!='a'||c.byte_at(c.pos+2)!='l'||c.byte_at(c.pos+3)!='s'||c.byte_at(c.pos+4)!='e') return false;
        c.pos += 5; vtype = T_FALSE;
      } else if (b == 'n') {
        if (c.end - c.pos < 4) return false;
        if (c.byte_at(c.pos+1)!='u'||c.byte_at(c.pos+2)!='l'||c.byte_at(c.pos+3)!='l') return false;
        c.pos += 4; vtype = T_NULL;
      } else if (b == '-' || (b >= '0' && b <= '9')) {
        NumOut n = parse_json_number(c);
        if (!n.ok) return false;
        vtype = T_NUM; vnum = n.v;
      } else {
        return false;
      }

      if (vtype != T_MISSING) {
        if (cur_capture && arr_depth == 0)
          fv.set(cur_slot, vtype, voff, vlen, vnum);
        if (depth == 0) { top_type = (top_type == T_MISSING) ? vtype : top_type; }
      }
      expect_value = false;
      continue;
    }

    if (depth == 0) {
      c.skip_ws();
      return c.eof();
    }
    c.skip_ws();
    if (c.eof()) return false;
    uint8_t b = c.next();
    bool in_arr = (is_arr_bits >> (depth - 1)) & 1u;
    if (in_arr) {
      if (b == ',') { expect_value = true; cur_capture = false; cur_slot = -1; continue; }
      if (b == ']') {
        depth--; arr_depth--;
        {
          int cs = (depth < SLOT_DEPTH)
                       ? (int)((cont_slot >> (5 * depth)) & 31ull) : 31;
          if (cs != 31) fv.set_len(cs, c.pos - fv.get_soff(cs));
        }
        cur_sig = (depth < SIG_DEPTH) ? sig_stack_at(depth) : 0;
        continue;
      }
      return false;
    } else {
      if (b == ',') {
        c.skip_ws();
        uint64_t parent = (depth - 1 < SIG_DEPTH) ? sig_stack_at(depth - 1) : 0;
        uint64_t ksig;
        if (!parse_key(parent, depth == 1, ksig)) return false;
        c.skip_ws();
        if (c.eof() || c.next() != ':') return false;
        cur_sig = ksig;
        cur_slot = (arr_depth == 0) ? match_slot(ksig) : -1;
        cur_capture = cur_slot >= 0;
        expect_value = true;
        continue;
      }
      if (b == '}') {
        depth--;
        {
          int cs = (depth < SLOT_DEPTH)
                       ? (int)((cont_slot >> (5 * depth)) & 31ull) : 31;
          if (cs != 31) fv.set_len(cs, c.pos - fv.get_soff(cs));
        }
        cur_sig = (depth < SIG_DEPTH) ? sig_stack_at(depth) : 0;
        continue;
      }
      return false;
    }
  }
}


template <class BS>
DN_HD_INLINE int eval_leaf(const PlanView& P, BS BV, const FV& fv,
                           int op, int slot, int cidx) {
  uint8_t ft = fv.get_type(slot);
  if (ft == T_MISSING) return -1;

  int ckind = P.const_meta[cidx * 6 + 0];
  uint32_t coff = (uint32_t)P.const_meta[cidx * 6 + 1];
  uint32_t clen = (uint32_t)P.const_meta[cidx * 6 + 2];
  int cdvalid = P.const_meta[cidx * 6 + 3];
  double cdval = P.const_dvals[cidx];

  if (op == OP_EQ || op == OP_NE) {
    bool eq = false;
    if (ft == T_NULL) {
      eq = (ckind == CONST_NULL);
    } else if (ckind == CONST_NULL) {
      eq = false;
    } else if (ft == T_TRUE || ft == T_FALSE || ft == T_NUM) {
      double fnum = (ft == T_NUM) ? fv.get_num(slot) : (ft == T_TRUE ? 1.0 : 0.0);
      if (ckind == CONST_NUM) eq = (fnum == cdval);
      else eq = cdvalid && (fnum == cdval);
    } else if (ft == T_STR) {
      if (ckind == CONST_STR) {
        uint32_t fo = fv.get_soff(slot), fl = fv.get_slen(slot);
        if (fl == clen) {
          eq = true;
          for (uint32_t k = 0; k < fl; k++)
            if (BV.at(fo + k) != P.const_bytes[coff + k]) { eq = false; break; }
        }
        if (!eq) {
          uint32_t co2 = (uint32_t)P.const_meta[cidx * 6 + 4];
          uint32_t cl2 = (uint32_t)P.const_meta[cidx * 6 + 5];
          if (cl2 != 0 && fl == cl2) {
            eq = true;
            for (uint32_t k = 0; k < fl; k++)
              if (BV.at(fo + k) != P.const_bytes[co2 + k]) { eq = false; break; }
          }
        }
        if (!eq && span_has_backslash(BV, fo, fl))
          eq = unesc_cmp(BV, fo, fl, P.const_bytes + coff, clen) == 0;
      } else {
        double fn = js_to_number(BV, fv.get_soff(slot), fv.get_slen(slot));
        eq = (fn == fn) && (fn == cdval);
      }
    } else {
      eq = false;
    }
    return (op == OP_EQ) ? (eq ? 1 : 0) : (eq ? 0 : 1);
  }

  if (ft == T_STR && ckind == CONST_STR) {
    uint32_t fo = fv.get_soff(slot), fl = fv.get_slen(slot);
    int cmp = 0;
    if (span_has_backslash(BV, fo, fl)) {
      cmp = unesc_cmp(BV, fo, fl, P.const_bytes + coff, clen);
      if (cmp == -2) cmp = 0;
    } else {
      uint32_t n = fl < clen ? fl : clen;
      for (uint32_t k = 0; k < n; k++) {
        uint8_t a = BV.at(fo + k), b = P.const_bytes[coff + k];
        if (a != b) { cmp = a < b ? -1 : 1; break; }
      }
      if (cmp == 0) cmp = (fl < clen) ? -1 : (fl > clen ? 1 : 0);
    }
    switch (op) {
      case OP_LT: return cmp < 0;
      case OP_LE: return cmp <= 0;
      case OP_GT: return cmp > 0;
      default:    return cmp >= 0;
    }
  }
  double x, y;
  if (ft == T_NUM) x = fv.get_num(slot);
  else if (ft == T_NULL) x = 0.0;
  else if (ft == T_TRUE) x = 1.0;
  else if (ft == T_FALSE) x = 0.0;
  else if (ft == T_STR) x = js_to_number(BV, fv.get_soff(slot), fv.get_slen(slot));
  else x = __builtin_nan("");
  if (ckind == CONST_NUM) y = cdval;
  else if (ckind == CONST_NULL) y = 0.0;
  else y = cdvalid ? cdval : __builtin_nan("");
  if (x != x || y != y) return 0;
  switch (op) {
    case OP_LT: return x < y;
    case OP_LE: return x <= y;
    case OP_GT: return x > y;
    default:    return x >= y;
  }
}

template <class BS>
DN_HD_INLINE int eval_predicate(const PlanView& P, BS BV,
                                const FV& fv, int prog_id) {
  int idx = P.prog_bounds[prog_id * 2 + 0];
  uint64_t stk[PRED_STACK];
  int sp = 0;
  int result;
  while (true) {
    int op = P.prog_nodes[idx * 4 + 0];
    if (op == OP_AND || op == OP_OR) {
      if (sp >= PRED_STACK) return -1;
      stk[sp] = ((uint64_t)(op == OP_OR)
                  | ((uint64_t)P.prog_nodes[idx * 4 + 1] << 1)
                  | ((uint64_t)P.prog_nodes[idx * 4 + 3] << 32));
      sp++;
      idx++;
      continue;
    }
    if (op == OP_TRUE) {
      result = 1;
      idx = P.prog_nodes[idx * 4 + 3];
    } else {
      result = eval_leaf(P, BV, fv, op,
                         P.prog_nodes[idx * 4 + 1],
                         P.prog_nodes[idx * 4 + 2]);
      idx = P.prog_nodes[idx * 4 + 3];
    }
    while (sp > 0) {
      if (result == -1) return -1;
      uint64_t f = stk[sp - 1];
      bool is_or = f & 1;
      uint32_t remaining = (uint32_t)(f >> 1) & 0x7FFFFF;
      bool sc = (!is_or && result == 0) || (is_or && result == 1);
      remaining--;
      if (sc || remaining == 0) {
        idx = (int)(f >> 32);
        sp--;
      } else {
        stk[sp - 1] = (f & 0xFFFFFFFF00000001ull)
                      | ((uint64_t)remaining << 1);
        break;
      }
    }
    if (sp == 0) return result;
  }
}

}
```

dragnet_amd/ops/hip/scan_tables.h:

```cpp
#pragma once
#include "scan_record.h"

namespace dn {

#define DEV __device__ __forceinline__

constexpr int LDS_CACHE = 128;

template <typename T>
DEV T atomic_load_relaxed(const T* p) {
  return __hip_atomic_load(p, __ATOMIC_RELAXED, __HIP_MEMORY_SCOPE_AGENT);
}
template <typename T>
DEV void atomic_store_relaxed(T* p, T v) {
  __hip_atomic_store(p, v, __ATOMIC_RELAXED, __HIP_MEMORY_SCOPE_AGENT);
}
DEV void drain_stores() {
  asm volatile("s_waitcnt vmcnt(0)" ::: "memory");
}


template <class BS>
DEV uint64_t hash_bytes(BS BV, uint32_t off, uint32_t len) {
  uint64_t h = FNV_OFFSET;
  for (uint32_t k = 0; k < len; k++) h = fnv1a_byte(h, BV.at(off + k));
  return mix64(h ^ len);
}

template <class BS>
DEV uint32_t intern_string(const StrDict& D, BS BV,
                           uint32_t off, uint32_t len) {
  uint64_t h = hash_bytes(BV, off, len);
  uint32_t mask = D.nslots - 1;
  uint32_t s = (uint32_t)h & mask;
  for (uint32_t probes = 0; probes < D.nslots; probes++, s = (s + 1) & mask) {
    while (true) {
      uint32_t st = atomic_load_relaxed(&D.state[s]);
      if (st == SLOT_READY) {
        if (atomic_load_relaxed(&D.hash[s]) != h) break;
        uint32_t o2 = atomic_load_relaxed(&D.off[s]);
        uint32_t l2 = atomic_load_relaxed(&D.len[s]);
        if (l2 != len) break;
        bool same = true;
        for (uint32_t k = 0; k < len; k++)
          if (D.data[o2 + k] != BV.at(off + k)) { same = false; break; }
        if (same) return atomic_load_relaxed(&D.id[s]);
        break;
      }
      if (st == SLOT_EMPTY) {
        uint32_t prev = atomicCAS(&D.state[s], SLOT_EMPTY, SLOT_CLAIMED);
        if (prev == SLOT_EMPTY) {
          uint32_t o = atomicAdd(D.data_used, (len + 7u) & ~7u);
          if (o + len > D.data_cap) return 0xFFFFFFFFu;
          for (uint32_t k = 0; k < len; k++)
            atomic_store_relaxed(&D.data[o + k], BV.at(off + k));
          uint32_t myid = atomicAdd(D.next_id, 1u);
          atomic_store_relaxed(&D.hash[s], h);
          atomic_store_relaxed(&D.off[s], o);
          atomic_store_relaxed(&D.len[s], len);
          atomic_store_relaxed(&D.id[s], myid);
          drain_stores();
          atomic_store_relaxed(&D.state[s], SLOT_READY);
          return myid;
        }
        continue;
      }
      __builtin_amdgcn_s_sleep(1);
    }
  }
  return 0xFFFFFFFFu;
}

DEV uint64_t number_hash(uint64_t bits) {
  return mix64(bits ^ 0x9E3779B97F4A7C15ull);
}

DEV uint32_t intern_number(const NumDict& D, double v) {
  if (v == 0.0) v = 0.0;
  uint64_t bits = __double_as_longlong(v);
  uint64_t h = number_hash(bits);
  uint32_t mask = D.nslots - 1;
  uint32_t s = (uint32_t)h & mask;
  for (uint32_t probes = 0; probes < D.nslots; probes++, s = (s + 1) & mask) {
    while (true) {
      uint32_t st = atomic_load_relaxed(&D.state[s]);
      if (st == SLOT_READY) {
        if (atomic_load_relaxed(&D.bits[s]) != bits) break;
        return atomic_load_relaxed(&D.id[s]);
      }
      if (st == SLOT_EMPTY) {
        uint32_t prev = atomicCAS(&D.state[s], SLOT_EMPTY, SLOT_CLAIMED);
        if (prev == SLOT_EMPTY) {
          uint32_t myid = atomicAdd(D.next_id, 1u);
          atomic_store_relaxed(&D.bits[s], bits);
          atomic_store_relaxed(&D.id[s], myid);
          drain_stores();
          atomic_store_relaxed(&D.state[s], SLOT_READY);
          return myid;
        }
        continue;
      }
      __builtin_amdgcn_s_sleep(1);
    }
  }
  return 0xFFFFFFFFu;
}


DEV uint64_t agg_table_hash(const uint32_t* key, int nk) {
  uint64_t h = FNV_OFFSET;
  for (int k = 0; k < MAX_KEY; k++)
    h = mix64(h ^ (k < nk ? key[k] : 0u) ^ (uint64_t)(k + 1) * 0x9E3779B97F4A7C15ull);
  return h;
}

constexpr uint32_t AGG_MAX_PROBES = 4096u;

DEV bool agg_insert(const AggTable& T, const uint32_t* key, int nk,
                    double w) {
  uint64_t h = agg_table_hash(key, nk);
  uint32_t mask = T.nslots - 1;
  uint32_t s = (uint32_t)h & mask;
  for (uint32_t probes = 0; probes < AGG_MAX_PROBES; probes++, s = (s + 1) & mask) {
    while (true) {
      uint32_t st = atomic_load_relaxed(&T.state[s]);
      if (st == SLOT_READY) {
        bool same = true;
#pragma unroll
        for (int k = 0; k < MAX_KEY; k++)
          if (k < nk &&
              atomic_load_relaxed(&T.keys[s * MAX_KEY + k]) != key[k])
            same = false;
        if (same) { atomicAdd(&T.count[s], w); return true; }
        break;
      }
      if (st == SLOT_EMPTY) {
        uint32_t prev = atomicCAS(&T.state[s], SLOT_EMPTY, SLOT_CLAIMED);
        if (prev == SLOT_EMPTY) {
#pragma unroll
          for (int k = 0; k < MAX_KEY; k++)
            atomic_store_relaxed(&T.keys[s * MAX_KEY + k],
                                 k < nk ? key[k] : 0u);
          drain_stores();
          atomic_store_relaxed(&T.state[s], SLOT_READY);
          atomicAdd(&T.count[s], w);
          return true;
        }
        continue;
      }
      __builtin_amdgcn_s_sleep(1);
    }
  }
  return false;
}

DEV uint32_t agg_insert_slot(const AggTable& T, const uint32_t* key,
                             int nk) {
  uint64_t h = agg_table_hash(key, nk);
  uint32_t mask = T.nslots - 1;
  uint32_t s = (uint32_t)h & mask;
  uint32_t max_probes = 256;
  for (uint32_t probes = 0; probes < max_probes; probes++, s = (s + 1) & mask) {
    while (true) {
      uint32_t st = atomic_load_relaxed(&T.state[s]);
      if (st == SLOT_READY) {
        bool same = true;
#pragma unroll
        for (int k = 0; k < MAX_KEY; k++)
          if (k < nk &&
              atomic_load_relaxed(&T.keys[s * MAX_KEY + k]) != key[k])
            same = false;
        if (same) return s;
        break;
      }
      if (st == SLOT_EMPTY) {
        uint32_t prev = atomicCAS(&T.state[s], SLOT_EMPTY, SLOT_CLAIMED);
        if (prev == SLOT_EMPTY) {
#pragma unroll
          for (int k = 0; k < MAX_KEY; k++)
            atomic_store_relaxed(&T.keys[s * MAX_KEY + k],
                                 k < nk ? key[k] : 0u);
          drain_stores();
          atomic_store_relaxed(&T.state[s], SLOT_READY);
          return s;
        }
        continue;
      }
      __builtin_amdgcn_s_sleep(1);
    }
  }
  return 0xFFFFFFFFu;
}

DEV bool agg_add(const AggTable& T, const uint32_t* key, int nk,
                 double w, unsigned long long* gflag) {
  if (T.partial != nullptr) {
    if (atomic_load_relaxed(gflag) != 0ull) return false;
    uint32_t s = agg_insert_slot(T, key, nk);
    if (s == 0xFFFFFFFFu) {
      atomicAdd(gflag, 1ull);
      return false;
    }
    atomicAdd(&T.partial[(size_t)(blockIdx.x % T.prows) * T.nslots + s],
              w);
    return true;
  }
  return agg_insert(T, key, nk, w);
}


struct LdsCacheEntry {
  uint64_t hash;
  uint32_t metric;
  uint32_t key[MAX_KEY];
  double count;
};

struct LdsLayout {
  size_t fv_soff, fv_slen, fv_type, cache, lcnt, synth, sig, tile, total;
  __host__ __device__ __forceinline__
  LdsLayout(int nf, int nm, int ns, bool parse_state) {
    size_t off = 0;
    fv_soff = off; off += (size_t)nf * BLOCK * sizeof(uint32_t);
    fv_slen = off; off += (size_t)nf * BLOCK * sizeof(uint32_t);
    fv_type = off; off += (size_t)nf * BLOCK * sizeof(uint8_t);
    off = (off + 15) & ~(size_t)15;
    cache = off; off += (size_t)LDS_CACHE * sizeof(LdsCacheEntry);
    lcnt = off;
    off += (size_t)(C_GLOBAL_N + nm * CM_N) * sizeof(unsigned long long);
    synth = sig = off;
    if (parse_state) {
      off += (size_t)ns * BLOCK * sizeof(double);
      sig = off; off += (size_t)SIG_DEPTH * BLOCK * sizeof(uint64_t);
    }
    off = (off + 15) & ~(size_t)15;
    tile = off;
    total = off + 64;
  }
};


template <class BS>
DEV bool encode_key_col(const StrDict& sdict, const NumDict& ndict, BS BV,
                       uint8_t t, double num, uint32_t so, uint32_t sl,
                       int bucket, double step, uint32_t& code,
                        bool& drop, bool& overflow) {
  if (bucket != BUCKET_NONE) {
    if (t == T_STR) {
      num = js_to_number(BV, so, sl);
      if (!(num == num) || num == __builtin_inf() ||
          num == -__builtin_inf())
        { drop = true; return false; }
      t = T_NUM;
    }
    if (t != T_NUM || !finite_num(num)) { drop = true; return false; }
    double ordf = bucket_ordinal(bucket, num, step);
    if (ord_is_small(ordf)) {
      code = make_code(TAG_ORD, (uint32_t)((int)ordf + ORD_BIAS));
    } else {
      uint32_t id = intern_number(ndict, ordf);
      if (id == 0xFFFFFFFFu) { overflow = true; return false; }
      code = make_code(TAG_NUM, id);
    }
  } else if (t == T_MISSING) {
    code = make_code(TAG_SPECIAL, SPECIAL_UNDEF);
  } else if (t == T_NULL) {
    code = make_code(TAG_SPECIAL, SPECIAL_NULL);
  } else if (t == T_TRUE) {
    code = make_code(TAG_SPECIAL, SPECIAL_TRUE);
  } else if (t == T_FALSE) {
    code = make_code(TAG_SPECIAL, SPECIAL_FALSE);
  } else if (t == T_OBJ) {
    code = make_code(TAG_SPECIAL, SPECIAL_OBJECT);
  } else if (t == T_ARR) {
    uint32_t id = intern_string(sdict, BV, so, sl);
    if (id == 0xFFFFFFFFu || id >= (1u << 27)) { overflow = true; return false; }
    code = make_code(TAG_SPECIAL, SPECIAL_ARRJSON | (id << 3));
  } else if (t == T_NUM) {
    uint32_t id = intern_number(ndict, num);
    if (id == 0xFFFFFFFFu) { overflow = true; return false; }
    code = make_code(TAG_NUM, id);
  } else {
    uint32_t id = intern_string(sdict, BV, so, sl);
    if (id == 0xFFFFFFFFu) { overflow = true; return false; }
    code = make_code(TAG_STR, id);
  }
  return true;
}

DEV uint64_t agg_key_hash(int m, const uint32_t* key) {
  uint64_t kh = mix64((uint64_t)m * 0x9E3779B97F4A7C15ull + 1);
  for (int k = 0; k < MAX_KEY; k++) kh = mix64(kh ^ key[k]);
  return kh == 0 ? 1 : kh;
}

template <int UNROLL>
DEV void lds_cache_add(LdsCacheEntry* cache, AggTable* tables,
                       unsigned long long* counters,
                       unsigned long long* lcnt, int m,
                       const uint32_t* key, int nk, uint64_t kh,
                       double weight) {
  bool cached = false;
  uint32_t ci = (uint32_t)kh & (LDS_CACHE - 1);
#pragma unroll UNROLL
  for (int attempt = 0; attempt < 8; attempt++) {
    unsigned long long prev = atomicCAS(
        (unsigned long long*)&cache[ci].hash, 0ull,
        (unsigned long long)kh);
    if (prev == 0) {
      cache[ci].metric = m;
      for (int k = 0; k < MAX_KEY; k++) cache[ci].key[k] = key[k];
      atomicAdd(&cache[ci].count, weight);
      cached = true;
      break;
    }
    if (prev == (unsigned long long)kh && cache[ci].metric == m) {
      bool same = true;
      for (int k = 0; k < MAX_KEY; k++)
        if (cache[ci].key[k] != key[k]) { same = false; break; }
      if (same) {
        atomicAdd(&cache[ci].count, weight);
        cached = true;
        break;
      }
    }
    ci = (ci + 1) & (LDS_CACHE - 1);
  }
  if (!cached) {
    if (!agg_add(tables[m], key, nk, weight, &counters[C_OVERFLOW]))
      atomicAdd(&lcnt[C_OVERFLOW], 1ull);
  }
}

DEV void block_agg_init(LdsCacheEntry* cache, unsigned long long* lcnt,
                        int ncnt) {
  for (int i = threadIdx.x; i < LDS_CACHE; i += BLOCK) {
    cache[i].hash = 0;
    cache[i].metric = 0;
    for (int k = 0; k < MAX_KEY; k++) cache[i].key[k] = 0;
    cache[i].count = 0.0;
  }
  for (int i = threadIdx.x; i < ncnt; i += BLOCK) lcnt[i] = 0;
  __syncthreads();
}

DEV void block_agg_flush(LdsCacheEntry* cache, unsigned long long* lcnt,
                         int ncnt, const PlanView& P, AggTable* tables,
                         unsigned long long* counters) {
  __syncthreads();
  for (int i = threadIdx.x; i < LDS_CACHE; i += BLOCK) {
    if (cache[i].hash != 0) {
      if (!agg_add(tables[cache[i].metric], cache[i].key,
                   P.metric_rows[cache[i].metric * 8 + 1],
                   cache[i].count, &counters[C_OVERFLOW]))
        atomicAdd(&lcnt[C_OVERFLOW], 1ull);
    }
  }
  __syncthreads();
  for (int i = threadIdx.x; i < ncnt; i += BLOCK) {
    if (lcnt[i]) atomicAdd(&counters[i], lcnt[i]);
  }
}

}
```

dragnet_amd/ops/hip/scan_text.h:

```cpp
#pragma once
#include "common.h"
#include "dec2dbl.h"

namespace dn {


DN_HD_INLINE uint64_t fnv1a_byte(uint64_t h, uint8_t b) {
  return (h ^ (uint64_t)b) * 0x100000001B3ull;
}
constexpr uint64_t FNV_OFFSET = 0xCBF29CE484222325ull;

DN_CONST_TABLE double P10_TBL[23] = {
  1e0,1e1,1e2,1e3,1e4,1e5,1e6,1e7,1e8,1e9,1e10,1e11,1e12,1e13,1e14,
  1e15,1e16,1e17,1e18,1e19,1e20,1e21,1e22};
DN_CONST_TABLE int DIM_TBL[12] = {
  31,28,31,30,31,30,31,31,30,31,30,31};

DN_HD_INLINE uint64_t mix64(uint64_t x) {
  x ^= x >> 33; x *= 0xFF51AFD7ED558CCDull;
  x ^= x >> 33; x *= 0xC4CEB9FE1A85EC53ull;
  x ^= x >> 33; return x;
}


struct Bytes {
  const uint8_t* mem;
  uint32_t bias;
  DN_HD_INLINE uint8_t at(uint32_t abs) const { return mem[abs - bias]; }
  DN_HD_INLINE uint64_t load8(uint32_t abs) const {
    uint64_t w;
    __builtin_memcpy(&w, mem + (abs - bias), 8);
    return w;
  }
};

template <int LG>
struct XBytesT {
  static constexpr uint32_t GRAN = 1u << LG;
  static constexpr uint32_t STRIDE = 64u << LG;
  const uint8_t* base;
  DN_HD_INLINE uint8_t at(uint32_t p) const {
    return base[(size_t)(p >> LG) * STRIDE + (p & (GRAN - 1u))];
  }
  DN_HD_INLINE uint64_t load8(uint32_t p) const {
    uint32_t o = p & (GRAN - 1u);
    const uint8_t* gp = base + (size_t)(p >> LG) * STRIDE;
    uint64_t w;
    if (o <= GRAN - 8) {
      __builtin_memcpy(&w, gp + o, 8);
      return w;
    }
    uint64_t lo, hi;
    __builtin_memcpy(&lo, gp + GRAN - 8, 8);
    __builtin_memcpy(&hi, gp + STRIDE, 8);
    uint32_t sh = (o - (GRAN - 8)) * 8;
    return (lo >> sh) | (hi << (64 - sh));
  }
};

template <class BS>
struct CursorT {
  BS B;
  uint32_t pos, end;
  uint64_t win, win2;
  uint32_t wbase;

  DN_HD_INLINE void init(BS b, uint32_t p, uint32_t e) {
    B = b; pos = p; end = e;
    wbase = p;
    win = B.load8(p);
    win2 = B.load8(p + 8);
  }
  DN_HD_INLINE uint8_t byte_at(uint32_t p) {
    uint32_t d = p - wbase;
    if (d >= 16u) {
      wbase = p;
      win = B.load8(p);
      win2 = B.load8(p + 8);
      d = 0;
    }
    uint64_t w = d < 8u ? win : win2;
    return (uint8_t)(w >> (8u * (d & 7u)));
  }
  DN_HD_INLINE bool eof() const { return pos >= end; }
  DN_HD_INLINE uint8_t peek() { return byte_at(pos); }
  DN_HD_INLINE uint8_t next() { return byte_at(pos++); }
  DN_HD_INLINE uint64_t word_at(uint32_t p) {
    uint32_t d = p - wbase;
    if (d > 8u) {
      wbase = p;
      win = B.load8(p);
      win2 = B.load8(p + 8);
      d = 0;
    }
    if (d == 0) return win;
    if (d == 8u) return win2;
    return (win >> (8u * d)) | (win2 << (64u - 8u * d));
  }
  DN_HD_INLINE void skip_ws() {
    while (pos < end) {
      uint8_t b = byte_at(pos);
      if (b == ' ' || b == '\t' || b == '\r' || b == '\n') pos++;
      else break;
    }
  }
};

DN_HD_INLINE uint64_t hz8(uint64_t v) {
  return (v - 0x0101010101010101ull) & ~v & 0x8080808080808080ull;
}

DN_HD_INLINE uint64_t str_special_mask(uint64_t w) {
  uint64_t q = hz8(w ^ 0x2222222222222222ull);
  uint64_t b = hz8(w ^ 0x5C5C5C5C5C5C5C5Cull);
  uint64_t c = hz8(w & 0xE0E0E0E0E0E0E0E0ull);
  return q | b | c;
}

template <class BS>
DN_HD_INLINE bool scan_string_fast(CursorT<BS>& c, uint32_t& off_out,
                                   uint32_t& len_out) {
  uint32_t off = c.pos, p = c.pos, end = c.end;
  while (true) {
    while (p + 8 <= end) {
      uint64_t w = c.B.load8(p);
      uint64_t m = str_special_mask(w);
      if (m == 0) { p += 8; continue; }
      p += ((uint32_t)DN_FFSLL((unsigned long long)m) - 1) >> 3;
      break;
    }
    if (p >= end) return false;
    uint8_t b = c.B.at(p);
    if (b == '"') {
      off_out = off; len_out = p - off; c.pos = p + 1;
      return true;
    }
    if (b == '\\') {
      p++;
      if (p >= end) return false;
      uint8_t e = c.B.at(p); p++;
      if (e == 'u') {
        if (p + 4 > end) return false;
        for (int k = 0; k < 4; k++) {
          uint8_t x = c.B.at(p + k);
          bool hex = (x >= '0' && x <= '9') || (x >= 'a' && x <= 'f') ||
                     (x >= 'A' && x <= 'F');
          if (!hex) return false;
        }
        p += 4;
      } else if (!(e == '"' || e == '\\' || e == '/' || e == 'b' ||
                   e == 'f' || e == 'n' || e == 'r' || e == 't')) {
        return false;
      }
      continue;
    }
    if (b < 0x20) return false;
    p++;
  }
}

constexpr uint64_t SIG_LENK = 0xFF51AFD7ED558CCDull;

DN_HD_INLINE uint64_t sig_mix(uint64_t x) {
  x ^= x >> 32;
  x *= 0xD6E8FEB86659FD93ull;
  return x ^ (x >> 32);
}
constexpr uint64_t SIG_LIT_MARK = 0xC2B2AE3D27D4EB4Full;

DN_HD_INLINE uint64_t sig_word(uint64_t sig, uint64_t w) {
  return sig_mix(sig ^ w);
}
DN_HD_INLINE uint64_t sig_fin(uint64_t sig, uint32_t len) {
  return sig_mix(sig ^ ((uint64_t)len * SIG_LENK));
}

template <class BS>
DN_HD_INLINE uint64_t sig_comp_finish(BS B, uint64_t sig, uint32_t hashed,
                                      uint32_t comp_s, uint32_t term) {
  uint32_t k = hashed;
  while (k < term) {
    uint64_t w = B.load8(k);
    uint32_t rem = term - k;
    if (rem < 8) w &= (~0ull) >> (8 * (8 - rem));
    sig = sig_mix(sig ^ w);
    k += 8;
  }
  return sig_fin(sig, term - comp_s);
}

template <class BS>
DN_HD_INLINE int scan_key_sig(CursorT<BS>& c, uint64_t parent,
                              uint64_t& sig_out, bool dot_splits) {
  uint32_t p = c.pos, end = c.end;
  uint32_t comp_s = p;
  uint32_t hashed = p;
  uint64_t sig = parent;
  bool saw_dot = false;
  while (true) {
    while (p + 8 <= end) {
      uint64_t w = c.B.load8(p);
      uint64_t m = str_special_mask(w);
      if (dot_splits) m |= hz8(w ^ 0x2E2E2E2E2E2E2E2Eull);
      if (m == 0) {
        if (p == hashed) {
          sig = sig_word(sig, w);
          hashed = p + 8;
        }
        p += 8;
        continue;
      }
      p += ((uint32_t)DN_FFSLL((unsigned long long)m) - 1) >> 3;
      break;
    }
    if (p >= end) return 0;
    uint8_t b = c.B.at(p);
    if (b == '"') {
      sig_out = sig_comp_finish(c.B, sig, hashed, comp_s, p);
      c.pos = p + 1;
      return saw_dot ? 2 : 1;
    }
    if (b == '.') {
      if (dot_splits) {
        sig = sig_comp_finish(c.B, sig, hashed, comp_s, p);
        comp_s = p + 1;
        hashed = p + 1;
        saw_dot = true;
      }
      p++;
      continue;
    }
    if (b == '\\') {
      c.pos = p;
      uint32_t o, l;
      if (!scan_string_fast(c, o, l)) return 0;
      sig_out = 0x1ull;
      return 1;
    }
    if (b < 0x20) return 0;
    p++;
  }
}


DN_HD_INLINE double scale10(uint64_t mant, long ex) {
  return dn_dec2dbl(mant, ex, P10_TBL);
}

struct NumOut { double v; bool ok; };

template <class BS>
DN_HD_INLINE int scan_digit_run(CursorT<BS>& c, uint64_t& mant, int& ndig,
                                int& extra) {
  int total = 0;
  while (!c.eof()) {
    uint64_t w = c.word_at(c.pos);
    uint64_t t = w ^ 0x3030303030303030ull;
    uint64_t nd = ((t + 0x7676767676767676ull) | t)
                  & 0x8080808080808080ull;
    uint32_t n = nd ? (((uint32_t)DN_FFSLL((long long)nd) - 1) >> 3)
                    : 8u;
    uint32_t avail = c.end - c.pos;
    if (n > avail) n = avail;
    if (n == 0) break;
    if (n == 8 && mant != 0 && ndig + 8 <= 19) {
      uint64_t pairs = (t * ((10ull << 8) + 1)) >> 8;
      uint64_t quads = ((pairs & 0x00FF00FF00FF00FFull)
                        * ((100ull << 16) + 1)) >> 16;
      uint64_t v8 = ((quads & 0x0000FFFF0000FFFFull)
                     * ((10000ull << 32) + 1)) >> 32;
      mant = mant * 100000000ull + (uint32_t)v8;
      ndig += 8;
    } else {
      for (uint32_t k = 0; k < n; k++) {
        uint32_t d = (uint32_t)(w >> (8 * k)) & 0xFF;
        if (ndig < 19) {
          mant = mant * 10u + (d - '0');
          ndig += (mant != 0);
        } else extra++;
      }
    }
    c.pos += n;
    total += (int)n;
    if (n < 8) break;
  }
  return total;
}

template <class BS>
DN_HD_INLINE NumOut parse_json_number(CursorT<BS>& c) {
  NumOut out; out.ok = false; out.v = 0.0;
  bool neg = false;
  if (!c.eof() && c.peek() == '-') { neg = true; c.pos++; }
  if (c.eof()) return out;
  uint64_t mant = 0;
  int ndig = 0, extra_exp = 0;
  uint8_t b = c.peek();
  if (b == '0') {
    c.pos++;
    if (!c.eof()) { uint8_t nb = c.peek(); if (nb >= '0' && nb <= '9') return out; }
  } else if (b >= '1' && b <= '9') {
    scan_digit_run(c, mant, ndig, extra_exp);
  } else {
    return out;
  }
  if (!c.eof() && c.peek() == '.') {
    c.pos++;
    int fdig = 0, fex = 0;
    fdig = scan_digit_run(c, mant, ndig, fex);
    extra_exp -= (fdig - fex);
    if (fdig == 0) return out;
  }
  int esign = 1; long e10 = 0;
  if (!c.eof() && (c.peek() == 'e' || c.peek() == 'E')) {
    c.pos++;
    if (!c.eof() && (c.peek() == '+' || c.peek() == '-')) {
      if (c.peek() == '-') esign = -1;
      c.pos++;
    }
    int edig = 0;
    while (!c.eof()) {
      uint8_t d = c.peek();
      if (d < '0' || d > '9') break;
      c.pos++;
      if (e10 < 100000) e10 = e10 * 10 + (d - '0');
      edig++;
    }
    if (edig == 0) return out;
  }
  long exp10 = esign * e10 + extra_exp;
  double v = scale10(mant, exp10);
  out.v = neg ? -v : v;
  out.ok = true;
  return out;
}

DN_HD_INLINE bool raw_ws(uint8_t b) {
  return b == ' ' || b == '\t' || b == '\r' || b == '\n' || b == '\f' ||
         b == '\v';
}

template <class BS>
DN_HD_INLINE uint32_t ws_escape_at(BS BV, uint32_t off, uint32_t p, uint32_t j,
                                   bool py_ws) {
  if (p + 2 > j || BV.at(off + p) != '\\') return 0;
  uint8_t e = BV.at(off + p + 1);
  if (e == 't' || e == 'n' || e == 'r' || e == 'f') return 2;
  if (e != 'u' || p + 6 > j) return 0;
  uint32_t cp = 0;
  for (int k = 2; k < 6; k++) {
    uint8_t x = BV.at(off + p + k);
    uint32_t d;
    if (x >= '0' && x <= '9') d = x - '0';
    else if (x >= 'a' && x <= 'f') d = x - 'a' + 10;
    else if (x >= 'A' && x <= 'F') d = x - 'A' + 10;
    else return 0;
    cp = cp * 16 + d;
  }
  bool ws = (cp >= 0x09 && cp <= 0x0D) || cp == 0x20 || cp == 0xA0 ||
            cp == 0x1680 || (cp >= 0x2000 && cp <= 0x200A) ||
            cp == 0x2028 || cp == 0x2029 || cp == 0x202F ||
            cp == 0x205F || cp == 0x3000 ||
            (py_ws ? ((cp >= 0x1C && cp <= 0x1F) || cp == 0x85)
                   : cp == 0xFEFF);
  return ws ? 6u : 0u;
}

template <class BS>
DN_HD_INLINE uint64_t trim_escaped_ws(BS BV, uint32_t off, uint32_t i,
                                      uint32_t j, bool py_ws) {
  while (i < j) {
    if (raw_ws(BV.at(off + i))) { i++; continue; }
    uint32_t n = ws_escape_at(BV, off, i, j, py_ws);
    if (n == 0) break;
    i += n;
  }
  while (j > i) {
    if (raw_ws(BV.at(off + j - 1))) { j--; continue; }
    uint32_t n = 0;
    if (j - i >= 2 && ws_escape_at(BV, off, j - 2, j, py_ws) == 2) n = 2;
    else if (j - i >= 6 && ws_escape_at(BV, off, j - 6, j, py_ws) == 6) n = 6;
    if (n == 0) break;
    uint32_t run = 0;
    for (uint32_t k = j - n; k > i && BV.at(off + k - 1) == '\\'; k--) run++;
    if (run & 1) break;
    j -= n;
  }
  return (uint64_t)i | ((uint64_t)j << 32);
}

template <class BS>
DN_HD_INLINE void trim_ws(BS BV, uint32_t off, uint32_t& i, uint32_t& j,
                          bool py_ws) {
  while (i < j && raw_ws(BV.at(off + i))) i++;
  while (j > i && raw_ws(BV.at(off + j - 1))) j--;
  if (j - i >= 2 &&
      (BV.at(off + i) == '\\' || BV.at(off + j - 2) == '\\' ||
       (j - i >= 6 && BV.at(off + j - 6) == '\\')))
  {
    uint64_t ij = trim_escaped_ws(BV, off, i, j, py_ws);
    i = (uint32_t)ij;
    j = (uint32_t)(ij >> 32);
  }
}

template <class BS>
DN_HD_INLINE double js_to_number(BS BV, uint32_t off, uint32_t len) {
  uint32_t i = 0, j = len;
  trim_ws(BV, off, i, j, false);
  if (i == j) return 0.0;
  const double NAN_ = __builtin_nan("");
  uint32_t p = i;
  bool neg = false;
  if (BV.at(off+p) == '+' || BV.at(off+p) == '-') { neg = BV.at(off+p) == '-'; p++; }
  if (p == j) return NAN_;
  if (BV.at(off+p) == 'I') {
    const char* inf = "Infinity";
    if (j - p == 8) {
      for (int k = 0; k < 8; k++) if (BV.at(off+p+k) != (uint8_t)inf[k]) return NAN_;
      return neg ? -__builtin_inf() : __builtin_inf();
    }
    return NAN_;
  }
  if (j - p > 2 && BV.at(off+p) == '0' &&
      (BV.at(off+p+1) == 'x' || BV.at(off+p+1) == 'X')) {
    if (p != i) return NAN_;
    uint64_t v = 0; int shift4 = 0; bool sticky = false;
    for (uint32_t k = p + 2; k < j; k++) {
      uint8_t b = BV.at(off+k);
      uint32_t d;
      if (b >= '0' && b <= '9') d = b - '0';
      else if (b >= 'a' && b <= 'f') d = b - 'a' + 10;
      else if (b >= 'A' && b <= 'F') d = b - 'A' + 10;
      else return NAN_;
      if (v >> 60) { shift4++; sticky |= (d != 0); }
      else v = v * 16u + d;
    }
    if (sticky) v |= 1;
    double r = (double)v;
    for (; shift4 > 0 && r < __builtin_inf(); shift4--) r *= 16.0;
    return r;
  }
  uint64_t mant = 0; int ndig = 0, extra = 0; bool any = false;
  while (p < j && BV.at(off+p) >= '0' && BV.at(off+p) <= '9') {
    if (ndig < 19) { mant = mant * 10 + (BV.at(off+p)-'0'); ndig += (mant != 0); }
    else extra++;
    p++; any = true;
  }
  if (p < j && BV.at(off+p) == '.') {
    p++;
    while (p < j && BV.at(off+p) >= '0' && BV.at(off+p) <= '9') {
      if (ndig < 19) { mant = mant * 10 + (BV.at(off+p)-'0'); ndig += (mant != 0); extra--; }
      p++; any = true;
    }
  }
  if (!any) return NAN_;
  long e10 = 0; int es = 1;
  if (p < j && (BV.at(off+p) == 'e' || BV.at(off+p) == 'E')) {
    p++;
    if (p < j && (BV.at(off+p) == '+' || BV.at(off+p) == '-')) {
      if (BV.at(off+p) == '-') es = -1;
      p++;
    }
    if (p >= j) return NAN_;
    while (p < j && BV.at(off+p) >= '0' && BV.at(off+p) <= '9') {
      if (e10 < 100000) e10 = e10 * 10 + (BV.at(off+p)-'0');
      p++;
    }
  }
  if (p != j) return NAN_;
  long ex = es * e10 + extra;
  double v = scale10(mant, ex);
  return neg ? -v : v;
}


DN_HD_INLINE bool finite_num(double v) {
  return __builtin_fabs(v) < __builtin_inf();
}

DN_HD_INLINE double bucket_ordinal(int kind, double num, double step) {
  if (kind == BUCKET_P2) {
    if (!(num >= 1.0)) return 0.0;
    uint64_t bits = DN_DOUBLE_AS_LL(num);
    return (double)((int)((bits >> 52) & 0x7FF) - 1023 + 1);
  }
  return __builtin_floor(num / step);
}

DN_HD_INLINE bool ord_is_small(double ordf) {
  return ordf >= -(double)ORD_BIAS && ordf < (double)ORD_BIAS;
}


DN_HD_INLINE long days_from_civil(long y, long m, long d) {
  y -= m <= 2;
  long era = (y >= 0 ? y : y - 399) / 400;
  long yoe = y - era * 400;
  long doy = (153 * (m + (m > 2 ? -3 : 9)) + 2) / 5 + d - 1;
  long doe = yoe * 365 + yoe / 4 - yoe / 100 + doy;
  return era * 146097 + doe - 719468;
}

struct DateOut { long long ms; bool ok; };

DN_HD_INLINE bool is_leap(long y) {
  return (y % 4 == 0) && ((y % 100 != 0) || (y % 400 == 0));
}

template <class BS>
DN_HD_INLINE DateOut parse_iso_ms(BS BV, uint32_t off, uint32_t len) {
  DateOut out; out.ok = false; out.ms = 0;
  uint32_t i = 0, j = len;
  trim_ws(BV, off, i, j, true);
  uint32_t p = i;
  auto digits = [&](int n, long& v) -> bool {
    v = 0;
    for (int k = 0; k < n; k++) {
      if (p >= j) return false;
      uint8_t b = BV.at(off+p);
      if (b < '0' || b > '9') return false;
      v = v * 10 + (b - '0');
      p++;
    }
    return true;
  };
  long year, month = 1, day = 1, hh = 0, mm = 0, ss = 0, ms = 0;
  if (!digits(4, year)) return out;
  bool have_time = false;
  if (p < j && BV.at(off+p) == '-') {
    p++;
    if (!digits(2, month)) return out;
    if (p < j && BV.at(off+p) == '-') {
      p++;
      if (!digits(2, day)) return out;
      if (p < j && (BV.at(off+p) == 'T' || BV.at(off+p) == ' ')) {
        p++;
        if (!digits(2, hh)) return out;
        if (p >= j || BV.at(off+p) != ':') return out;
        p++;
        if (!digits(2, mm)) return out;
        have_time = true;
        if (p < j && BV.at(off+p) == ':') {
          p++;
          if (!digits(2, ss)) return out;
          if (p < j && BV.at(off+p) == '.') {
            p++;
            int nd = 0; long frac = 0;
            while (p < j && BV.at(off+p) >= '0' && BV.at(off+p) <= '9' && nd < 9) {
              if (nd < 3) frac = frac * 10 + (BV.at(off+p) - '0');
              nd++; p++;
            }
            if (nd == 0) return out;
            while (nd < 3) { frac *= 10; nd++; }
            ms = frac;
          }
        }
      }
    }
  }
  long tz_off_min = 0;
  if (have_time && p < j) {
    uint8_t b = BV.at(off+p);
    if (b == 'Z') { p++; }
    else if (b == '+' || b == '-') {
      int sign = (b == '+') ? 1 : -1;
      p++;
      long th, tm;
      if (!digits(2, th)) return out;
      if (p < j && BV.at(off+p) == ':') p++;
      if (!digits(2, tm)) return out;
      tz_off_min = sign * (th * 60 + tm);
    }
  }
  if (p != j) return out;
  if (month < 1 || month > 12) return out;
  long dim = DIM_TBL[month-1] + ((month == 2 && is_leap(year)) ? 1 : 0);
  if (day < 1 || day > dim) return out;
  if (hh > 24 || mm > 59 || ss > 59) return out;
  if (hh == 24 && (mm || ss || ms)) return out;
  long days = days_from_civil(year, month, day);
  long long total = ((days * 24 + hh) * 60 + mm) * 60 + ss;
  out.ms = total * 1000 + ms - (long long)tz_off_min * 60000;
  out.ok = true;
  return out;
}


DN_HD_INLINE int hexval4(uint8_t x) {
  if (x >= '0' && x <= '9') return x - '0';
  if (x >= 'a' && x <= 'f') return x - 'a' + 10;
  if (x >= 'A' && x <= 'F') return x - 'A' + 10;
  return -1;
}

template <class BS>
DN_HD_INLINE int unesc_next(BS d, uint32_t fo, uint32_t fl,
                            uint32_t& i, uint32_t& out) {
  uint8_t b = d.at(fo + i);
  if (b != '\\') { i++; out = b; return 1; }
  if (i + 2 > fl) return 0;
  uint8_t e = d.at(fo + i + 1);
  i += 2;
  switch (e) {
    case '"':  out = '"';  return 1;
    case '\\': out = '\\'; return 1;
    case '/':  out = '/';  return 1;
    case 'b':  out = 8;    return 1;
    case 'f':  out = 12;   return 1;
    case 'n':  out = 10;   return 1;
    case 'r':  out = 13;   return 1;
    case 't':  out = 9;    return 1;
    case 'u':  break;
    default:   return 0;
  }
  if (i + 4 > fl) return 0;
  uint32_t cp = 0;
  for (int k = 0; k < 4; k++) {
    int h = hexval4(d.at(fo + i + k));
    if (h < 0) return 0;
    cp = cp * 16 + (uint32_t)h;
  }
  i += 4;
  if (cp >= 0xD800 && cp < 0xDC00 && i + 6 <= fl &&
      d.at(fo + i) == '\\' && d.at(fo + i + 1) == 'u') {
    uint32_t lo = 0;
    bool ok = true;
    for (int k = 0; k < 4; k++) {
      int h = hexval4(d.at(fo + i + 2 + k));
      if (h < 0) { ok = false; break; }
      lo = lo * 16 + (uint32_t)h;
    }
    if (ok && lo >= 0xDC00 && lo < 0xE000) {
      cp = 0x10000 + ((cp - 0xD800) << 10) + (lo - 0xDC00);
      i += 6;
    }
  }
  if (cp < 0x80) { out = cp; return 1; }
  if (cp < 0x800) {
    out = (0xC0 | (cp >> 6)) | ((0x80u | (cp & 63)) << 8);
    return 2;
  }
  if (cp < 0x10000) {
    out = (0xE0 | (cp >> 12)) | ((0x80u | ((cp >> 6) & 63)) << 8)
          | ((0x80u | (cp & 63)) << 16);
    return 3;
  }
  out = (0xF0 | (cp >> 18)) | ((0x80u | ((cp >> 12) & 63)) << 8)
        | ((0x80u | ((cp >> 6) & 63)) << 16)
        | ((0x80u | (cp & 63)) << 24);
  return 4;
}

template <class BS>
DN_HD_INLINE int unesc_cmp(BS d, uint32_t fo, uint32_t fl,
                           const uint8_t* cb, uint32_t cl) {
  uint32_t i = 0, j = 0;
  while (i < fl) {
    uint32_t pack;
    int n = unesc_next(d, fo, fl, i, pack);
    if (n == 0) return -2;
    for (int k = 0; k < n; k++) {
      uint8_t a = (uint8_t)(pack >> (8 * k));
      if (j >= cl) return 1;
      uint8_t b = cb[j++];
      if (a != b) return a < b ? -1 : 1;
    }
  }
  return (j == cl) ? 0 : -1;
}

template <class BS>
DN_HD_INLINE bool span_has_backslash(BS d, uint32_t fo, uint32_t fl) {
  for (uint32_t k = 0; k < fl; k++)
    if (d.at(fo + k) == '\\') return true;
  return false;
}

}
```

tools_dev/kernel_host_check.cpp:

```cpp
#include <cinttypes>
#include <cstdio>
#include <cstdlib>
#include <cstring>
#include <iostream>
#include <sstream>
#include <string>
#include <vector>

#include "scan_record.h"

using namespace dn;

static uint64_t bits_of(double v) {
  uint64_t b;
  std::memcpy(&b, &v, 8);
  return b;
}

static std::string unhex(const std::string& h) {
  std::string out;
  if (h == "-") return out;
  for (size_t i = 0; i + 1 < h.size(); i += 2)
    out.push_back((char)std::stoi(h.substr(i, 2), nullptr, 16));
  return out;
}

template <class BS> struct Staged;

template <> struct Staged<Bytes> {
  uint8_t* buf;
  Bytes src;
  explicit Staged(const std::string& rec) {
    size_t n = rec.size() + 1;
    size_t padded = (n + 16 + 15) & ~(size_t)15;
    buf = (uint8_t*)std::malloc(padded);
    std::memset(buf, '\n', padded);
    std::memcpy(buf, rec.data(), rec.size());
    src.mem = buf;
    src.bias = 0;
  }
  ~Staged() { std::free(buf); }
};

template <int LG> struct Staged<XBytesT<LG>> {
  uint8_t* buf;
  XBytesT<LG> src;
  explicit Staged(const std::string& rec) {
    const size_t GRAN = XBytesT<LG>::GRAN, STRIDE = XBytesT<LG>::STRIDE;
    size_t rows = (rec.size() + GRAN - 1) / GRAN;
    if (rows == 0) rows = 1;
    size_t total = rows * STRIDE + STRIDE;
    buf = (uint8_t*)std::malloc(total);
    std::memset(buf, '\n', total);
    for (size_t p = 0; p < rec.size(); p++)
      buf[(p >> LG) * STRIDE + (p & (GRAN - 1))] = (uint8_t)rec[p];
    src.base = buf;
  }
  ~Staged() { std::free(buf); }
};

struct Plan {
  std::vector<uint64_t> field_sigs;
  std::vector<int32_t> prog_nodes, prog_bounds, const_meta;
  std::vector<double> const_dvals;
  std::vector<uint8_t> const_bytes;
  bool dot_splits = false;
  PlanView P;
  std::vector<uint8_t> fv_type;
  std::vector<uint32_t> fv_soff, fv_slen;
  std::vector<uint64_t> sig_stack;

  void bind() {
    P.field_sigs = field_sigs.data();
    P.prog_nodes = prog_nodes.data();
    P.prog_bounds = prog_bounds.data();
    P.const_meta = const_meta.data();
    P.const_dvals = const_dvals.data();
    P.const_bytes = const_bytes.data();
    fv_type.assign((size_t)P.nf * BLOCK, T_MISSING);
    fv_soff.assign((size_t)P.nf * BLOCK, 0);
    fv_slen.assign((size_t)P.nf * BLOCK, 0);
    sig_stack.assign((size_t)SIG_DEPTH * BLOCK, 0);
  }
};

template <class BS>
static void do_record(Plan& pl, const std::string& rec) {
  Staged<BS> st(rec);
  pl.bind();
  FV fv;
  fv.type = pl.fv_type.data();
  fv.soff = pl.fv_soff.data();
  fv.slen = pl.fv_slen.data();
  fv.tid = 0;
  uint8_t top = T_MISSING;
  bool ok = parse_record(st.src, 0u, (uint32_t)rec.size(), pl.P, fv, top,
                         pl.sig_stack.data(), pl.dot_splits);
  if (!ok) { std::printf("0\n"); return; }
  std::printf("1 %d", (int)top);
  for (int f = 0; f < pl.P.nf; f++) {
    int t = fv.get_type(f);
    if (t == T_NUM)
      std::printf(" 4:%016" PRIx64, bits_of(fv.get_num(f)));
    else if (t == T_STR || t == T_OBJ || t == T_ARR)
      std::printf(" %d:%u:%u", t, fv.get_soff(f), fv.get_slen(f));
    else
      std::printf(" %d", t);
  }
  std::printf(" ;");
  int nprogs = (int)pl.prog_bounds.size() / 2;
  for (int p = 0; p < nprogs; p++)
    std::printf(" %d", eval_predicate(pl.P, st.src, fv, p));
  std::printf("\n");
}

template <class BS>
static int serve() {
  Plan pl;
  std::memset(&pl.P, 0, sizeof(pl.P));
  std::string line, mode, tok;
  while (std::getline(std::cin, line)) {
    std::istringstream in(line);
    if (!(in >> mode)) continue;
    if (mode == "dec2dbl") {
      unsigned long long mant; long ex;
      in >> mant >> ex;
      std::printf("%016" PRIx64 "\n",
                  bits_of(dn_dec2dbl((uint64_t)mant, ex, P10_TBL)));
    } else if (mode == "number") {
      in >> tok;
      std::string lit = unhex(tok);
      Staged<BS> st(lit);
      CursorT<BS> c;
      c.init(st.src, 0u, (uint32_t)lit.size());
      NumOut n = parse_json_number(c);
      std::printf("%s %016" PRIx64 " %u\n",
                  n.ok && c.pos == c.end ? "ok" : "invalid", bits_of(n.v),
                  c.pos);
    } else if (mode == "tonumber") {
      in >> tok;
      std::string s = unhex(tok);
      Staged<BS> st(s);
      std::printf("%016" PRIx64 "\n",
                  bits_of(js_to_number(st.src, 0u, (uint32_t)s.size())));
    } else if (mode == "date") {
      in >> tok;
      std::string s = unhex(tok);
      Staged<BS> st(s);
      DateOut d = parse_iso_ms(st.src, 0u, (uint32_t)s.size());
      if (d.ok) std::printf("ok %lld\n", d.ms);
      else std::printf("invalid\n");
    } else if (mode == "keysig") {
      int dot_splits;
      in >> dot_splits;
      uint64_t sig = FNV_OFFSET;
      bool ok = true;
      while (ok && (in >> tok)) {
        std::string key = unhex(tok) + "\"";
        Staged<BS> st(key);
        CursorT<BS> c;
        c.init(st.src, 0u, (uint32_t)key.size());
        uint64_t out = 0;
        ok = scan_key_sig(c, sig, out, dot_splits != 0) != 0;
        sig = out;
      }
      if (ok) std::printf("%016" PRIx64 "\n", sig);
      else std::printf("invalid\n");
    } else if (mode == "plan") {
      int ds;
      std::string bloom, fps;
      in >> ds >> pl.P.nf >> bloom >> fps;
      pl.dot_splits = ds != 0;
      pl.P.sig_bloom = std::stoull(bloom, nullptr, 16);
      pl.P.fields_parent_sig = std::stoull(fps, nullptr, 16);
    } else if (mode == "field_sigs") {
      pl.field_sigs.clear();
      while (in >> tok) pl.field_sigs.push_back(std::stoull(tok, nullptr, 16));
    } else if (mode == "const_dvals") {
      pl.const_dvals.clear();
      while (in >> tok) {
        uint64_t b = std::stoull(tok, nullptr, 16);
        double v;
        std::memcpy(&v, &b, 8);
        pl.const_dvals.push_back(v);
      }
    } else if (mode == "const_bytes") {
      in >> tok;
      std::string b = unhex(tok);
      pl.const_bytes.assign(b.begin(), b.end());
    } else if (mode == "prog_nodes" || mode == "prog_bounds" ||
               mode == "const_meta") {
      std::vector<int32_t>& v = mode == "prog_nodes" ? pl.prog_nodes
                              : mode == "prog_bounds" ? pl.prog_bounds
                                                      : pl.const_meta;
      v.clear();
      long x;
      while (in >> x) v.push_back((int32_t)x);
    } else if (mode == "record") {
      tok = "-";
      in >> tok;
      do_record<BS>(pl, unhex(tok));
    } else {
      std::fprintf(stderr, "unknown request: %s\n", mode.c_str());
      return 2;
    }
  }
  return 0;
}

int main(int argc, char** argv) {
  std::string src = argc > 1 ? argv[1] : "bytes";
  if (src == "bytes") return serve<Bytes>();
  if (src == "x5") return serve<XBytesT<5>>();
  if (src == "x6") return serve<XBytesT<6>>();
  if (src == "x7") return serve<XBytesT<7>>();
  std::fprintf(stderr, "usage: kernel_host_check <bytes|x5|x6|x7>\n");
  return 2;
}
```

Measured before the change: 248.8 million records/s.

## Add LDS-staged granule scan kernel and trim signature stack to plan depth

Sizes the per-thread key-signature stack in LDS to the deepest field path used by the plan instead of a fixed depth, and skips slot matching for keys deeper than that. Adds an optional scan kernel variant that stages record bytes into LDS in 32/64-byte granules via global_load_lds, selected by an environment variable. The trimmed stack reduces LDS per block, which may raise occupancy. The granule path adds complexity and an alignment requirement and is off by default.

Result: no change. 248.9 million records/s, median of 3 (+0.0%).

```diff
diff --git a/dragnet_amd/engine/gpu.py b/dragnet_amd/engine/gpu.py
--- a/dragnet_amd/engine/gpu.py
+++ b/dragnet_amd/engine/gpu.py
@@ -156,6 +156,7 @@
             nf_match=cplan.nf_match,
             sig_bloom=cplan.sig_bloom,
             fields_parent_sig=cplan.fields_parent_sig,
+            sig_levels=cplan.sig_levels,
             prog_nodes=dev_i32(progs),
             prog_bounds=dev_i32(bounds),
             const_meta=dev_i32(cplan.const_meta),
@@ -251,7 +252,7 @@
     def _submit(self, dev_data, start, end, index=None):
         pos, nlines = index or self._index(dev_data, start, end)
         if self.planner is None:
-            self.state.scan(dev_data, pos, nlines, start)
+            self.state.scan(dev_data, pos, nlines, start, _pad(end))
         else:
             self._scan_planned(dev_data, pos, nlines, start, end)
 
@@ -275,7 +276,8 @@
         a = 0
         while a < nrec:
             b = pl.next_range(a, nrec, start_of, self._measure, self.grow)
-            self.state.scan(dev_data, pos[a:b], nlines, start_of(a))
+            self.state.scan(dev_data, pos[a:b], nlines, start_of(a),
+                            _pad(end))
             a = b
 
     def _measure(self, names):
diff --git a/dragnet_amd/engine/plan.py b/dragnet_amd/engine/plan.py
--- a/dragnet_amd/engine/plan.py
+++ b/dragnet_amd/engine/plan.py
@@ -80,6 +80,14 @@
     for comp in path.split("."):
         sig = comp_into(sig, comp.encode("utf-8"))
     return sig
+
+
+SIG_DEPTH = 6
+
+
+def sig_levels(paths):
+    deepest = max([len(p.split(".")) for p in paths] or [1])
+    return min(deepest, SIG_DEPTH)
 
 
 class PlanError(Exception):
@@ -358,6 +366,8 @@
     plan.fields_slot = fields_slot
     fps = path_sig("fields") if data_format == "json-skinner" else 0
     plan.fields_parent_sig = fps - (1 << 64) if fps >= (1 << 63) else fps
+    plan.sig_levels = sig_levels(
+        [p if raw else prefix + p for p, raw in fields.paths])
     plan.ds_prog = ds_prog
     plan.data_format = data_format
     return plan
diff --git a/dragnet_amd/ops/hip/common.h b/dragnet_amd/ops/hip/common.h
--- a/dragnet_amd/ops/hip/common.h
+++ b/dragnet_amd/ops/hip/common.h
@@ -114,6 +114,7 @@
   int value_slot;
   int fields_slot;
   uint64_t fields_parent_sig;
+  int sig_levels;
 };
 
 struct ScanArgs {
@@ -123,6 +124,7 @@
   uint32_t pos_cap;
   uint32_t first_start;
   uint32_t tile_cap;
+  uint32_t data_limit;
   PlanView P;
   AggTable* tables;
   StrDict sdict;
diff --git a/dragnet_amd/ops/hip/ext.hip b/dragnet_amd/ops/hip/ext.hip
--- a/dragnet_amd/ops/hip/ext.hip
+++ b/dragnet_amd/ops/hip/ext.hip
@@ -39,10 +39,14 @@
   return v ? atoi(v) : dflt;
 }
 
-size_t lds_bytes(int64_t nf, int64_t nm, int64_t ns, bool columnar) {
-  return LdsLayout((int)nf, (int)nm, columnar ? 0 : (int)ns, !columnar)
+size_t lds_bytes(int64_t nf, int64_t nm, int64_t ns, bool columnar,
+                 int64_t sig_levels, int64_t granule) {
+  return LdsLayout((int)nf, (int)nm, columnar ? 0 : (int)ns, !columnar,
+                   (int)sig_levels, (int)granule)
       .total;
 }
+
+constexpr size_t LDS_FOUR_BLOCKS = LDS_MAX / 4;
 
 using ScanKernel = void (*)(ScanArgs);
 
@@ -55,6 +59,10 @@
     case 6: return scan_kernel_mw<6>;
     default: return scan_kernel;
   }
+}
+
+ScanKernel granule_kernel(int gran) {
+  return gran == 32 ? scan_kernel_g<4, 5> : scan_kernel_g<4, 6>;
 }
 
 ScanKernel xpose_kernel(int mw, int xg) {
@@ -162,6 +170,9 @@
     P.fields_slot = py::cast<int>(plan["fields_slot"]);
     P.fields_parent_sig =
         (uint64_t)py::cast<int64_t>(plan["fields_parent_sig"]);
+    P.sig_levels = py::cast<int>(plan["sig_levels"]);
+    TORCH_CHECK(P.sig_levels >= 1 && P.sig_levels <= SIG_DEPTH,
+                "plan sig_levels must be 1..", SIG_DEPTH);
     args_.data_format_skinner = py::cast<bool>(plan["skinner"]) ? 1 : 0;
 
     for (auto& t : owned_) CHECK_GPU(t);
@@ -190,7 +201,7 @@
     linear_ = linear_kernel(mw);
     xpose_ = xpose_kernel(mw, env_int("DRAGNET_XGRAN", 64));
 
-    lds_ = lds_bytes(P.nf, P.nm, P.ns, false);
+    lds_ = lds_bytes(P.nf, P.nm, P.ns, false, P.sig_levels, 0);
     TORCH_CHECK(lds_ <= LDS_MAX, "plan needs too much LDS: ", lds_);
     int tile_req = env_int("DRAGNET_LDS_STAGE", 0);
     if (tile_req != 0) {
@@ -201,20 +212,42 @@
       if (tile_cap_ < 24 * 1024) tile_cap_ = 0;
     }
     args_.tile_cap = (uint32_t)tile_cap_;
+
+    int gran = env_int("DRAGNET_GRANULE", 0);
+    TORCH_CHECK(gran == 0 || gran == 32 || gran == 64,
+                "DRAGNET_GRANULE must be 0, 32 or 64");
+    if (tile_cap_ != 0 || mw != 4) gran = 0;
+    while (gran != 0 && lds_bytes(P.nf, P.nm, P.ns, false, P.sig_levels,
+                                  gran) > LDS_FOUR_BLOCKS)
+      gran = gran == 64 ? 32 : 0;
+    granule_ = gran;
+    lds_linear_ = lds_;
+    if (gran != 0) {
+      linear_ = granule_kernel(gran);
+      lds_linear_ = lds_bytes(P.nf, P.nm, P.ns, false, P.sig_levels, gran);
+    }
   }
 
   void scan(torch::Tensor data, torch::Tensor nl_pos,
-            torch::Tensor nlines, int64_t first_start) {
+            torch::Tensor nlines, int64_t first_start,
+            int64_t padded_len) {
     CHECK_GPU(data);
     CHECK_GPU(nl_pos);
+    if (padded_len < 0) padded_len = data.numel();
+    TORCH_CHECK(padded_len <= data.numel() &&
+                    padded_len <= (int64_t)0xFFFFFFFFll,
+                "padded_len exceeds the data tensor");
     ScanArgs A = args_;
     A.data = (const uint8_t*)data.data_ptr();
+    TORCH_CHECK(granule_ == 0 || ((uintptr_t)A.data & 63u) == 0,
+                "scan data must be 64-byte aligned");
+    A.data_limit = (uint32_t)padded_len & ~15u;
     A.nl_pos = (const uint32_t*)nl_pos.data_ptr();
     A.nlines_ptr = (const uint32_t*)nlines.data_ptr();
     A.pos_cap = (uint32_t)nl_pos.numel();
     A.first_start = (uint32_t)first_start;
     launch("scan_kernel", linear_, dim3(grid_for(A.pos_cap)), dim3(BLOCK),
-           lds_ + tile_cap_, A);
+           lds_linear_ + tile_cap_, A);
   }
 
   void scan_xpose(torch::Tensor xdata, torch::Tensor wave_base,
@@ -346,6 +379,9 @@
 
   torch::Tensor counters() const { return counters_; }
 
+  int64_t granule() const { return granule_; }
+  int64_t lds_linear() const { return (int64_t)(lds_linear_ + tile_cap_); }
+
 
   torch::Tensor occupancy() {
     std::vector<torch::Tensor> parts;
@@ -464,7 +500,7 @@
     A.P = column_plan();
     TORCH_CHECK(col_descs.numel() == (int64_t)(A.P.nf * sizeof(ColDesc)),
                 "col_descs does not match the plan's field count");
-    L.lds = lds_bytes(A.P.nf, A.P.nm, 0, true);
+    L.lds = lds_bytes(A.P.nf, A.P.nm, 0, true, SIG_DEPTH, 0);
     TORCH_CHECK(L.lds <= LDS_MAX, what, " plan needs too much LDS");
     A.nrows = (uint32_t)nrows;
     A.values = (const double*)values.data_ptr();
@@ -573,7 +609,8 @@
   ScanArgs args_ = {};
   std::vector<AggTable> tables_;
   ScanKernel linear_ = nullptr, xpose_ = nullptr;
-  size_t lds_ = 0, tile_cap_ = 0;
+  size_t lds_ = 0, lds_linear_ = 0, tile_cap_ = 0;
+  int granule_ = 0;
 };
 
 }
@@ -585,6 +622,7 @@
   m.def("col_descs_host", &dn::col_descs_host);
   m.def("lds_bytes", &dn::lds_bytes, py::arg("nf"), py::arg("nm"),
         py::arg("ns") = 0, py::arg("columnar") = false,
+        py::arg("sig_levels") = (int)dn::SIG_DEPTH, py::arg("granule") = 0,
         "dynamic LDS bytes of a scan / columnar launch (host only)");
   py::class_<dn::ScanState>(m, "ScanState")
       .def(py::init<py::dict, int64_t, int64_t, int64_t, bool>(),
@@ -593,6 +631,7 @@
            py::arg("dense"))
       .def("scan", &dn::ScanState::scan, py::arg("data"),
            py::arg("nl_pos"), py::arg("nlines"), py::arg("first_start"),
+           py::arg("padded_len") = -1,
            "fused NDJSON scan over one chunk")
       .def("scan_xpose", &dn::ScanState::scan_xpose, py::arg("xdata"),
            py::arg("wave_base"), py::arg("rec_len"), py::arg("n_slots"))
@@ -612,6 +651,8 @@
            "payload bytes, number ids]")
       .def("sizes", &dn::ScanState::sizes)
       .def_property_readonly("counters", &dn::ScanState::counters)
+      .def_property_readonly("granule", &dn::ScanState::granule)
+      .def_property_readonly("lds_linear", &dn::ScanState::lds_linear)
       .def("grow_agg", &dn::ScanState::grow_agg, py::arg("metric"),
            py::arg("new_slots"),
            "rehash one metric's table into a larger zeroed one")
@@ -620,4 +661,5 @@
       .def("grow_ndict", &dn::ScanState::grow_ndict, py::arg("new_slots"));
   m.attr("MAX_KEY") = (int)dn::MAX_KEY;
   m.attr("MAX_FIELDS") = (int)dn::MAX_FIELDS;
-}
+  m.attr("SIG_DEPTH") = (int)dn::SIG_DEPTH;
+}
diff --git a/dragnet_amd/ops/hip/hd.h b/dragnet_amd/ops/hip/hd.h
--- a/dragnet_amd/ops/hip/hd.h
+++ b/dragnet_amd/ops/hip/hd.h
@@ -16,7 +16,9 @@
 #define DN_LL_AS_DOUBLE(x) __longlong_as_double(x)
 #define DN_TID() ((uint32_t)threadIdx.x)
 #define DN_CONST_TABLE __device__ __constant__
+#define DN_LDS __attribute__((address_space(3)))
 #else
+#define DN_LDS
 #define DN_FFSLL(x) __builtin_ffsll((long long)(x))
 #define DN_DOUBLE_AS_LL(x) __builtin_bit_cast(long long, (double)(x))
 #define DN_LL_AS_DOUBLE(x) __builtin_bit_cast(double, (long long)(x))
diff --git a/dragnet_amd/ops/hip/scan_kernels.hip b/dragnet_amd/ops/hip/scan_kernels.hip
--- a/dragnet_amd/ops/hip/scan_kernels.hip
+++ b/dragnet_amd/ops/hip/scan_kernels.hip
@@ -187,7 +187,7 @@
   }
 }
 
-template <int XP>
+template <int XP, int GL = 0>
 DEV void scan_kernel_body(char* smem, ScanArgs A);
 
 __launch_bounds__(BLOCK)
@@ -220,6 +220,15 @@
 template __global__ void scan_kernel_x<5, 6>(ScanArgs);
 template __global__ void scan_kernel_x<4, 5>(ScanArgs);
 template __global__ void scan_kernel_x<4, 7>(ScanArgs);
+
+template <int MW, int GLG>
+__launch_bounds__(BLOCK, MW)
+__global__ void scan_kernel_g(ScanArgs A) {
+  extern __shared__ __attribute__((aligned(16))) char smem3[];
+  scan_kernel_body<0, GLG>(smem3, A);
+}
+template __global__ void scan_kernel_g<4, 6>(ScanArgs);
+template __global__ void scan_kernel_g<4, 5>(ScanArgs);
 
 #define synth_val_at(si) synth_lds[(si) * BLOCK + threadIdx.x]
 
@@ -369,12 +378,13 @@
   }
 }
 
-template <int XP>
+template <int XP, int GL>
 DEV void scan_kernel_body(char* smem, ScanArgs A) {
   const PlanView& P = A.P;
   const int nf = P.nf;
 
-  const LdsLayout L(nf, P.nm, P.ns, true);
+  const LdsLayout L(nf, P.nm, P.ns, true, P.sig_levels,
+                    GL ? (1 << GL) : 0);
   LdsCacheEntry* cache = reinterpret_cast<LdsCacheEntry*>(smem + L.cache);
   unsigned long long* lcnt =
       reinterpret_cast<unsigned long long*>(smem + L.lcnt);
@@ -405,6 +415,23 @@
                          synth_lds);
         }
       }
+    }
+  } else if constexpr (GL != 0) {
+    uint32_t nlines = *A.nlines_ptr;
+    if (nlines > A.pos_cap) nlines = A.pos_cap;
+    GranBytesT<GL> BV;
+    BV.mem = A.data;
+    BV.limit = A.data_limit;
+    BV.slot = (DN_LDS uint8_t*)(smem + L.gran)
+              + (threadIdx.x >> 6) * GranBytesT<GL>::WAVE_BYTES
+              + (threadIdx.x & 63u) * 16u;
+    const uint32_t stride_g = gridDim.x * BLOCK;
+    for (uint32_t r = blockIdx.x * BLOCK + threadIdx.x; r < nlines;
+         r += stride_g) {
+      uint32_t start = r ? A.nl_pos[r - 1] + 1 : A.first_start;
+      uint32_t end = A.nl_pos[r];
+      process_record(BV, start, end, A, P, fv, lcnt, cache, sig_lds,
+                     synth_lds);
     }
   } else {
   uint32_t nlines = *A.nlines_ptr;
diff --git a/dragnet_amd/ops/hip/scan_record.h b/dragnet_amd/ops/hip/scan_record.h
--- a/dragnet_amd/ops/hip/scan_record.h
+++ b/dragnet_amd/ops/hip/scan_record.h
@@ -52,6 +52,8 @@
   uint64_t cur_sig = 0;
   bool cur_capture = false;
   int cur_slot = -1;
+
+  const int sig_levels = P.sig_levels;
 
   c.skip_ws();
   if (c.eof()) return false;
@@ -104,7 +106,7 @@
             cont_slot = (cont_slot & ~(31ull << (5 * depth)))
                         | (cs << (5 * depth));
           }
-          if (depth < SIG_DEPTH) sig_stack_at(depth) = cur_sig;
+          if (depth < sig_levels) sig_stack_at(depth) = cur_sig;
           is_arr_bits &= ~(1ull << depth);
           depth++;
           uint64_t ksig;
@@ -112,7 +114,8 @@
           c.skip_ws();
           if (c.eof() || c.next() != ':') return false;
           cur_sig = ksig;
-          cur_slot = (arr_depth == 0) ? match_slot(ksig) : -1;
+          cur_slot = (arr_depth == 0 && depth <= sig_levels)
+                         ? match_slot(ksig) : -1;
           cur_capture = cur_slot >= 0;
           continue;
         }
@@ -135,7 +138,7 @@
             cont_slot = (cont_slot & ~(31ull << (5 * depth)))
                         | (cs << (5 * depth));
           }
-          if (depth < SIG_DEPTH) sig_stack_at(depth) = cur_sig;
+          if (depth < sig_levels) sig_stack_at(depth) = cur_sig;
           is_arr_bits |= (1ull << depth);
           depth++;
           arr_depth++;
@@ -192,20 +195,21 @@
                        ? (int)((cont_slot >> (5 * depth)) & 31ull) : 31;
           if (cs != 31) fv.set_len(cs, c.pos - fv.get_soff(cs));
         }
-        cur_sig = (depth < SIG_DEPTH) ? sig_stack_at(depth) : 0;
+        cur_sig = (depth < sig_levels) ? sig_stack_at(depth) : 0;
         continue;
       }
       return false;
     } else {
       if (b == ',') {
         c.skip_ws();
-        uint64_t parent = (depth - 1 < SIG_DEPTH) ? sig_stack_at(depth - 1) : 0;
+        uint64_t parent = (depth - 1 < sig_levels) ? sig_stack_at(depth - 1) : 0;
         uint64_t ksig;
         if (!parse_key(parent, depth == 1, ksig)) return false;
         c.skip_ws();
         if (c.eof() || c.next() != ':') return false;
         cur_sig = ksig;
-        cur_slot = (arr_depth == 0) ? match_slot(ksig) : -1;
+        cur_slot = (arr_depth == 0 && depth <= sig_levels)
+                       ? match_slot(ksig) : -1;
         cur_capture = cur_slot >= 0;
         expect_value = true;
         continue;
@@ -217,7 +221,7 @@
                        ? (int)((cont_slot >> (5 * depth)) & 31ull) : 31;
           if (cs != 31) fv.set_len(cs, c.pos - fv.get_soff(cs));
         }
-        cur_sig = (depth < SIG_DEPTH) ? sig_stack_at(depth) : 0;
+        cur_sig = (depth < sig_levels) ? sig_stack_at(depth) : 0;
         continue;
       }
       return false;
diff --git a/dragnet_amd/ops/hip/scan_tables.h b/dragnet_amd/ops/hip/scan_tables.h
--- a/dragnet_amd/ops/hip/scan_tables.h
+++ b/dragnet_amd/ops/hip/scan_tables.h
@@ -217,9 +217,11 @@
 };
 
 struct LdsLayout {
-  size_t fv_soff, fv_slen, fv_type, cache, lcnt, synth, sig, tile, total;
+  size_t fv_soff, fv_slen, fv_type, cache, lcnt, synth, sig, gran, tile,
+      total;
   __host__ __device__ __forceinline__
-  LdsLayout(int nf, int nm, int ns, bool parse_state) {
+  LdsLayout(int nf, int nm, int ns, bool parse_state,
+            int sig_levels = SIG_DEPTH, int gran_bytes = 0) {
     size_t off = 0;
     fv_soff = off; off += (size_t)nf * BLOCK * sizeof(uint32_t);
     fv_slen = off; off += (size_t)nf * BLOCK * sizeof(uint32_t);
@@ -228,10 +230,12 @@
     cache = off; off += (size_t)LDS_CACHE * sizeof(LdsCacheEntry);
     lcnt = off;
     off += (size_t)(C_GLOBAL_N + nm * CM_N) * sizeof(unsigned long long);
-    synth = sig = off;
+    synth = sig = gran = off;
     if (parse_state) {
       off += (size_t)ns * BLOCK * sizeof(double);
-      sig = off; off += (size_t)SIG_DEPTH * BLOCK * sizeof(uint64_t);
+      sig = off; off += (size_t)sig_levels * BLOCK * sizeof(uint64_t);
+      off = (off + 15) & ~(size_t)15;
+      gran = off; off += (size_t)gran_bytes * BLOCK;
     }
     off = (off + 15) & ~(size_t)15;
     tile = off;
diff --git a/dragnet_amd/ops/hip/scan_text.h b/dragnet_amd/ops/hip/scan_text.h
--- a/dragnet_amd/ops/hip/scan_text.h
+++ b/dragnet_amd/ops/hip/scan_text.h
@@ -58,12 +58,31 @@
   }
 };
 
+template <int LG>
+struct GranBytesT {
+  static constexpr uint32_t GRAN = 1u << LG;
+  static constexpr uint32_t NCH = GRAN / 16;
+  static constexpr uint32_t ROW = 64 * 16;
+  static constexpr uint32_t WAVE_BYTES = NCH * ROW;
+  const uint8_t* mem;
+  uint32_t limit;
+  DN_LDS uint8_t* slot;
+  DN_HD_INLINE uint8_t at(uint32_t abs) const { return mem[abs]; }
+  DN_HD_INLINE uint64_t load8(uint32_t abs) const {
+    uint64_t w;
+    __builtin_memcpy(&w, mem + abs, 8);
+    return w;
+  }
+};
+
 template <class BS>
 struct CursorT {
   BS B;
   uint32_t pos, end;
   uint64_t win, win2;
   uint32_t wbase;
+
+  DN_HD_INLINE BS& seq() { return B; }
 
   DN_HD_INLINE void init(BS b, uint32_t p, uint32_t e) {
     B = b; pos = p; end = e;
@@ -97,6 +116,107 @@
     if (d == 8u) return win2;
     return (win >> (8u * d)) | (win2 << (64u - 8u * d));
   }
+  DN_HD_INLINE void skip_ws() {
+    while (pos < end) {
+      uint8_t b = byte_at(pos);
+      if (b == ' ' || b == '\t' || b == '\r' || b == '\n') pos++;
+      else break;
+    }
+  }
+};
+
+template <int LG>
+struct CursorT<GranBytesT<LG>> {
+  using BS = GranBytesT<LG>;
+  static constexpr uint32_t GRAN = BS::GRAN;
+  BS B;
+  uint32_t pos, end;
+  uint32_t gbase;
+
+  DN_HD_INLINE CursorT& seq() { return *this; }
+
+  DN_HD_INLINE void fill() {
+#if defined(__HIP_DEVICE_COMPILE__)
+    DN_LDS uint8_t* row = B.slot - (DN_TID() & 63u) * 16u;
+    asm volatile("s_waitcnt lgkmcnt(0)" ::: "memory");
+#pragma unroll
+    for (uint32_t j = 0; j < BS::NCH; j++) {
+      uint32_t a = gbase + j * 16u;
+      if (a < B.limit)
+        __builtin_amdgcn_global_load_lds(
+            (const __attribute__((address_space(1))) void*)(B.mem + a),
+            (DN_LDS void*)(row + j * BS::ROW), 16, 0, 0);
+    }
+    asm volatile("s_waitcnt vmcnt(0)" ::: "memory");
+#else
+    for (uint32_t j = 0; j < BS::NCH; j++) {
+      uint32_t a = gbase + j * 16u;
+      if (a < B.limit) __builtin_memcpy(B.slot + j * BS::ROW, B.mem + a, 16);
+    }
+#endif
+  }
+  DN_HD_INLINE void seek(uint32_t p) {
+    gbase = p & ~(GRAN - 1u);
+    fill();
+  }
+  DN_HD_INLINE static uint32_t col(uint32_t d) {
+    return (d >> 4) * BS::ROW + (d & 15u);
+  }
+  DN_HD_INLINE uint64_t lds8(uint32_t d) const {
+#if defined(__HIP_DEVICE_COMPILE__)
+    return *reinterpret_cast<DN_LDS const uint64_t*>(B.slot + col(d));
+#else
+    uint64_t w;
+    __builtin_memcpy(&w, B.slot + col(d), 8);
+    return w;
+#endif
+  }
+
+  DN_HD_INLINE void init(BS b, uint32_t p, uint32_t e) {
+    B = b; pos = p; end = e;
+    seek(p);
+  }
+  DN_HD_INLINE uint8_t byte_at(uint32_t p) {
+    uint32_t d = p - gbase;
+    if (d >= GRAN) {
+      if (p < gbase) return B.at(p);
+      seek(p);
+      d = p - gbase;
+    }
+    return B.slot[col(d)];
+  }
+  DN_HD_INLINE bool eof() const { return pos >= end; }
+  DN_HD_INLINE uint8_t peek() { return byte_at(pos); }
+  DN_HD_INLINE uint8_t next() { return byte_at(pos++); }
+  DN_HD_INLINE uint64_t word_at(uint32_t p) {
+    uint32_t d = p - gbase;
+    if (d >= GRAN) {
+      if (p < gbase) return B.load8(p);
+      seek(p);
+      d = p - gbase;
+    }
+    if (d >= GRAN - 8u) return B.load8(p);
+    uint32_t q = d & ~7u, sh = (d & 7u) * 8u;
+    return (lds8(q) >> sh) | ((lds8(q + 8u) << 1) << (63u - sh));
+  }
+  DN_HD_INLINE void chunk_at(uint32_t p, uint64_t& lo, uint64_t& hi) {
+    uint32_t d = p - gbase;
+    if (d >= GRAN) {
+      seek(p);
+      d = p - gbase;
+    }
+#if defined(__HIP_DEVICE_COMPILE__)
+    typedef uint64_t u64x2 __attribute__((ext_vector_type(2)));
+    u64x2 v = *reinterpret_cast<DN_LDS const u64x2*>(
+        B.slot + (d >> 4) * BS::ROW);
+    lo = v.x; hi = v.y;
+#else
+    __builtin_memcpy(&lo, B.slot + (d >> 4) * BS::ROW, 8);
+    __builtin_memcpy(&hi, B.slot + (d >> 4) * BS::ROW + 8, 8);
+#endif
+  }
+  DN_HD_INLINE uint8_t at(uint32_t p) { return byte_at(p); }
+  DN_HD_INLINE uint64_t load8(uint32_t p) { return word_at(p); }
   DN_HD_INLINE void skip_ws() {
     while (pos < end) {
       uint8_t b = byte_at(pos);
@@ -159,6 +279,60 @@
   }
 }
 
+DN_HD_INLINE uint64_t plain_below(uint64_t w, uint32_t k) {
+  uint64_t keep = ~0ull << (8u * k);
+  return (w & keep) | (0x6161616161616161ull & ~keep);
+}
+
+template <int LG>
+DN_HD_INLINE bool scan_string_fast(CursorT<GranBytesT<LG>>& c,
+                                   uint32_t& off_out, uint32_t& len_out) {
+  uint32_t off = c.pos, p = c.pos, end = c.end;
+  while (true) {
+    if (p >= end) return false;
+    uint32_t cb = p & ~15u, k = p - cb;
+    uint64_t lo, hi;
+    c.chunk_at(p, lo, hi);
+    if (k >= 8) {
+      lo = 0x6161616161616161ull;
+      hi = plain_below(hi, k - 8u);
+    } else {
+      lo = plain_below(lo, k);
+    }
+    uint64_t w = lo, m = str_special_mask(lo);
+    uint32_t at = cb;
+    if (m == 0) {
+      w = hi; m = str_special_mask(hi); at = cb + 8u;
+    }
+    if (m == 0) { p = cb + 16u; continue; }
+    uint32_t i = ((uint32_t)DN_FFSLL((unsigned long long)m) - 1) >> 3;
+    p = at + i;
+    if (p >= end) return false;
+    uint8_t b = (uint8_t)(w >> (8u * i));
+    if (b == '"') {
+      off_out = off; len_out = p - off; c.pos = p + 1;
+      return true;
+    }
+    if (b != '\\') return false;
+    p++;
+    if (p >= end) return false;
+    uint8_t e = c.byte_at(p); p++;
+    if (e == 'u') {
+      if (p + 4 > end) return false;
+      for (int x4 = 0; x4 < 4; x4++) {
+        uint8_t x = c.byte_at(p + x4);
+        bool hex = (x >= '0' && x <= '9') || (x >= 'a' && x <= 'f') ||
+                   (x >= 'A' && x <= 'F');
+        if (!hex) return false;
+      }
+      p += 4;
+    } else if (!(e == '"' || e == '\\' || e == '/' || e == 'b' ||
+                 e == 'f' || e == 'n' || e == 'r' || e == 't')) {
+      return false;
+    }
+  }
+}
+
 constexpr uint64_t SIG_LENK = 0xFF51AFD7ED558CCDull;
 
 DN_HD_INLINE uint64_t sig_mix(uint64_t x) {
@@ -175,8 +349,8 @@
   return sig_mix(sig ^ ((uint64_t)len * SIG_LENK));
 }
 
-template <class BS>
-DN_HD_INLINE uint64_t sig_comp_finish(BS B, uint64_t sig, uint32_t hashed,
+template <class SEQ>
+DN_HD_INLINE uint64_t sig_comp_finish(SEQ& B, uint64_t sig, uint32_t hashed,
                                       uint32_t comp_s, uint32_t term) {
   uint32_t k = hashed;
   while (k < term) {
@@ -192,6 +366,7 @@
 template <class BS>
 DN_HD_INLINE int scan_key_sig(CursorT<BS>& c, uint64_t parent,
                               uint64_t& sig_out, bool dot_splits) {
+  auto& S = c.seq();
   uint32_t p = c.pos, end = c.end;
   uint32_t comp_s = p;
   uint32_t hashed = p;
@@ -199,7 +374,7 @@
   bool saw_dot = false;
   while (true) {
     while (p + 8 <= end) {
-      uint64_t w = c.B.load8(p);
+      uint64_t w = S.load8(p);
       uint64_t m = str_special_mask(w);
       if (dot_splits) m |= hz8(w ^ 0x2E2E2E2E2E2E2E2Eull);
       if (m == 0) {
@@ -214,15 +389,15 @@
       break;
     }
     if (p >= end) return 0;
-    uint8_t b = c.B.at(p);
+    uint8_t b = S.at(p);
     if (b == '"') {
-      sig_out = sig_comp_finish(c.B, sig, hashed, comp_s, p);
+      sig_out = sig_comp_finish(S, sig, hashed, comp_s, p);
       c.pos = p + 1;
       return saw_dot ? 2 : 1;
     }
     if (b == '.') {
       if (dot_splits) {
-        sig = sig_comp_finish(c.B, sig, hashed, comp_s, p);
+        sig = sig_comp_finish(S, sig, hashed, comp_s, p);
         comp_s = p + 1;
         hashed = p + 1;
         saw_dot = true;
diff --git a/tools_dev/kernel_host_check.cpp b/tools_dev/kernel_host_check.cpp
--- a/tools_dev/kernel_host_check.cpp
+++ b/tools_dev/kernel_host_check.cpp
@@ -40,6 +40,26 @@
     src.bias = 0;
   }
   ~Staged() { std::free(buf); }
+};
+
+template <int LG> struct Staged<GranBytesT<LG>> {
+  uint8_t* buf;
+  uint8_t* lds;
+  GranBytesT<LG> src;
+  explicit Staged(const std::string& rec) {
+    size_t n = rec.size() + 1;
+    size_t padded = (n + 16 + 15) & ~(size_t)15;
+    buf = (uint8_t*)std::malloc(padded);
+    std::memset(buf, '\n', padded);
+    std::memcpy(buf, rec.data(), rec.size());
+    size_t win = (GranBytesT<LG>::NCH - 1) * GranBytesT<LG>::ROW + 16;
+    lds = (uint8_t*)std::malloc(win);
+    std::memset(lds, 0xEE, win);
+    src.mem = buf;
+    src.limit = (uint32_t)padded;
+    src.slot = lds;
+  }
+  ~Staged() { std::free(buf); std::free(lds); }
 };
 
 template <int LG> struct Staged<XBytesT<LG>> {
@@ -80,7 +100,7 @@
     fv_type.assign((size_t)P.nf * BLOCK, T_MISSING);
     fv_soff.assign((size_t)P.nf * BLOCK, 0);
     fv_slen.assign((size_t)P.nf * BLOCK, 0);
-    sig_stack.assign((size_t)SIG_DEPTH * BLOCK, 0);
+    sig_stack.assign((size_t)P.sig_levels * BLOCK, 0);
   }
 };
 
@@ -118,6 +138,7 @@
 static int serve() {
   Plan pl;
   std::memset(&pl.P, 0, sizeof(pl.P));
+  pl.P.sig_levels = SIG_DEPTH;
   std::string line, mode, tok;
   while (std::getline(std::cin, line)) {
     std::istringstream in(line);
@@ -170,6 +191,7 @@
       int ds;
       std::string bloom, fps;
       in >> ds >> pl.P.nf >> bloom >> fps;
+      if (!(in >> pl.P.sig_levels)) pl.P.sig_levels = SIG_DEPTH;
       pl.dot_splits = ds != 0;
       pl.P.sig_bloom = std::stoull(bloom, nullptr, 16);
       pl.P.fields_parent_sig = std::stoull(fps, nullptr, 16);
@@ -214,6 +236,9 @@
   if (src == "x5") return serve<XBytesT<5>>();
   if (src == "x6") return serve<XBytesT<6>>();
   if (src == "x7") return serve<XBytesT<7>>();
-  std::fprintf(stderr, "usage: kernel_host_check <bytes|x5|x6|x7>\n");
+  if (src == "g5") return serve<GranBytesT<5>>();
+  if (src == "g6") return serve<GranBytesT<6>>();
+  std::fprintf(stderr,
+               "usage: kernel_host_check <bytes|x5|x6|x7|g5|g6>\n");
   return 2;
 }
```
